# lswzjuer/pytorch-quantity

Measured on NVIDIA B200. Metric: calib images/sec (hist+KL), higher is better.
Workload: dtype f32

## Files before the change

include/pq_sm100.h:

```cpp
#ifndef PQ_SM100_H
#define PQ_SM100_H

#include <stddef.h>
#include <stdint.h>

#ifdef __cplusplus
extern "C" {
#endif

typedef void *pq_stream_t;

#define PQ_VERSION 201

#define PQ_OK 0
#define PQ_EINVAL (-1)
#define PQ_EUNSUPPORTED (-2)
#define PQ_EALIGN (-3)
#define PQ_ETOOMANY (-4)

#define PQ_HIST_BINS 2048
#define PQ_HIST_BINS_MAX 8192
#define PQ_KL_TARGET_BIN 128
#define PQ_KL_CANDIDATES (PQ_HIST_BINS - PQ_KL_TARGET_BIN)
#define PQ_MAX_SEGMENTS 256

int pq_version(void);
const char *pq_error_string(int code);

int pq_absmax_multi_f32(const float *const *xs_host, const uint64_t *ns_host, int k,
                        uint32_t *max_bits, pq_stream_t stream);

int pq_absmax_per_channel_f32(const float *x, uint64_t outer, int channels, uint64_t inner,
                              uint32_t *max_bits, pq_stream_t stream);

int pq_conv_epilogue_f32(float *y, const float *bias, int N, int C, uint64_t hw, float *relu_out,
                         uint32_t *max_slot, pq_stream_t stream);
int pq_eltwise_add_f32(const float *a, const float *b, float *z, size_t n, float *relu_out, uint32_t *max_slot,
                       pq_stream_t stream);

int pq_hist2048_multi_f32(const float *const *xs_host, const uint64_t *ns_host,
                          const float *intervals_host, int k, long long *hist,
                          pq_stream_t stream);

size_t pq_kl_workspace_doubles(void);
int pq_kl_search_f64(const double *counts, int k, double *workspace, double *kl,
                     int *threshold, pq_stream_t stream);

int pq_hist_multi_f32(const float *const *xs_host, const uint64_t *ns_host, const float *intervals_host,
                      int k, int nbins, long long *hist, pq_stream_t stream);
size_t pq_kl_workspace_doubles_n(int nbins);
int pq_kl_search_n_f64(const double *counts, int k, int nbins, double *workspace, double *kl,
                       int *threshold, pq_stream_t stream);

int pq_fakequant_f32(const float *x, float *y, size_t n, int bit, float lo, float hi,
                     int dequant, pq_stream_t stream);

int pq_add_clamp_f32(const float *a, const float *b, float *y, size_t n, float lo, float hi,
                     pq_stream_t stream);

int pq_rshift_f32(const float *x, float *y, size_t n, int rs, float lo, float hi, pq_stream_t stream);

int pq_clamp_scale_f32(const float *x, float *y, size_t n, float lo, float hi, float scale,
                       pq_stream_t stream);

int pq_quantize_nchw_to_nhwc_s8(const float *x, int8_t *q, int N, int C, int H, int W, int c_pad,
                                int ib, pq_stream_t stream);

int pq_quantize_im2col_s8(const float *x, int8_t *a, int N, int C, int H, int W, int R, int S,
                          int stride_h, int stride_w, int pad_h, int pad_w, int kp, int ib,
                          pq_stream_t stream);

int pq_quantize_nchw_to_padded_nhwc8_s8(const float *x, int8_t *q, int N, int C, int H, int W, int pad_h,
                                        int pad_w, int Hp, int Wp, int ib, pq_stream_t stream);

typedef struct pq_conv_desc {
    int N, H, W, C;
    int K;
    int R, S;
    int stride_h, stride_w, pad_h, pad_w;
    int P, Q;
    int rs;
    int ob;
    int dil_h, dil_w;
} pq_conv_desc;

#define PQ_FLAG_RELU 1
#define PQ_FLAG_BIAS_FOLDED 2
#define PQ_FLAG_NO_WINDOWS 4

int pq_gemm_s8(const int8_t *a, const int8_t *w, const int32_t *bias_q, int M, int N, int K, int rs, int ob, int hw,
               int flags, float *out_f32, int8_t *out_s8, pq_stream_t stream);
int pq_conv2d_s8(const int8_t *x_nhwc, const int8_t *w_krsc, const int32_t *bias_q, const pq_conv_desc *desc_host,
                 int flags, float *out_f32_nchw, int8_t *out_s8_nhwc, pq_stream_t stream);

int pq_bias_fold_s32(const int32_t *bias_q, int n, int rs, int32_t *out, pq_stream_t stream);

int pq_quantize_nchw_to_s2d16_s8(const float *x, int8_t *q, int N, int C, int H, int W, int pad_t, int pad_l,
                                 int Hp2, int Wp2, int ib, pq_stream_t stream);

int pq_conv2d_smallc_s8(const int8_t *xp, const int8_t *w_krs8, const int32_t *bias_q,
                        const pq_conv_desc *desc_host, int Hp, int Wp, int flags, float *out_f32_nchw,
                        int8_t *out_s8_nhwc, pq_stream_t stream);

int pq_avgpool_global_nhwc_f32(const void *x, int is16, int bit, int relu, int N, int HW, int C, float *out,
                               pq_stream_t stream);

int pq_relu_s8(const int8_t *x, int8_t *y, size_t n, pq_stream_t stream);

int pq_maxpool_nhwc_s8(const int8_t *x, int8_t *y, int N, int H, int W, int C, int k, int stride, int pad,
                       int relu, pq_stream_t stream);

int pq_add_requant(const void *a, int a_is16, int a_bit, int a_relu, const void *b, int b_is16, int b_bit,
                   int b_relu, size_t n, int flags, int16_t *out16, int8_t *out8, int q_bit, pq_stream_t stream);

#define PQ_CONCAT_MAX_SOURCES 8
typedef struct pq_concat_src {
    const void *ptr;
    int is16;
    int channels;
    int bit;
    int relu;
} pq_concat_src;
int pq_concat_requant_s8(const pq_concat_src *srcs_host, int k, size_t pixels, int q_bit, int c_out_pad,
                         int8_t *out, pq_stream_t stream);

typedef struct pq_add_desc {
    const void *shortcut;
    int shortcut_is16, shortcut_bit, shortcut_relu;
    int out_relu;
    int q_bit;
    int16_t *out16;
    int8_t *out8;
} pq_add_desc;
int pq_conv2d_s8_add(const int8_t *x_nhwc, const int8_t *w_krsc, const int32_t *bias_q, const pq_conv_desc *desc_host,
                     const pq_add_desc *add_host, int flags, pq_stream_t stream);

#ifdef __cplusplus
}
#endif
#endif
```

pytorch-quantity_b200/common/quantity/_native.py:

```python
import ctypes
import os

import numpy as np
import torch

_PKG_ROOT = os.path.dirname(os.path.dirname(os.path.dirname(os.path.abspath(__file__))))
LIB_PATH = os.path.join(_PKG_ROOT, "lib", "libpq_sm100.so")

HIST_BINS = 2048
HIST_BINS_MAX = 8192
KL_TARGET_BIN = 128
KL_CANDIDATES = HIST_BINS - KL_TARGET_BIN
MAX_SEGMENTS = 256
PQ_VERSION = 201

_vp, _i, _sz, _f = ctypes.c_void_p, ctypes.c_int, ctypes.c_size_t, ctypes.c_float
SYMBOLS = {
    "pq_version": (_i, []),
    "pq_error_string": (ctypes.c_char_p, [_i]),
    "pq_absmax_multi_f32": (_i, [_vp, _vp, _i, _vp, _vp]),
    "pq_absmax_per_channel_f32": (_i, [_vp, ctypes.c_uint64, _i, ctypes.c_uint64, _vp, _vp]),
    "pq_conv_epilogue_f32": (_i, [_vp, _vp, _i, _i, ctypes.c_uint64, _vp, _vp, _vp]),
    "pq_eltwise_add_f32": (_i, [_vp, _vp, _vp, _sz, _vp, _vp, _vp]),
    "pq_hist2048_multi_f32": (_i, [_vp, _vp, _vp, _i, _vp, _vp]),
    "pq_kl_workspace_doubles": (_sz, []),
    "pq_kl_search_f64": (_i, [_vp, _i, _vp, _vp, _vp, _vp]),
    "pq_hist_multi_f32": (_i, [_vp, _vp, _vp, _i, _i, _vp, _vp]),
    "pq_kl_workspace_doubles_n": (_sz, [_i]),
    "pq_kl_search_n_f64": (_i, [_vp, _i, _i, _vp, _vp, _vp, _vp]),
    "pq_fakequant_f32": (_i, [_vp, _vp, _sz, _i, _f, _f, _i, _vp]),
    "pq_add_clamp_f32": (_i, [_vp, _vp, _vp, _sz, _f, _f, _vp]),
    "pq_rshift_f32": (_i, [_vp, _vp, _sz, _i, _f, _f, _vp]),
    "pq_clamp_scale_f32": (_i, [_vp, _vp, _sz, _f, _f, _f, _vp]),
    "pq_quantize_nchw_to_nhwc_s8": (_i, [_vp, _vp, _i, _i, _i, _i, _i, _i, _vp]),
    "pq_quantize_im2col_s8": (_i, [_vp, _vp] + [_i] * 12 + [_vp]),
    "pq_quantize_nchw_to_padded_nhwc8_s8": (_i, [_vp, _vp] + [_i] * 9 + [_vp]),
    "pq_conv2d_smallc_s8": (_i, [_vp, _vp, _vp, _vp, _i, _i, _i, _vp, _vp, _vp]),
    "pq_quantize_nchw_to_s2d16_s8": (_i, [_vp, _vp] + [_i] * 9 + [_vp]),
    "pq_gemm_s8": (_i, [_vp, _vp, _vp, _i, _i, _i, _i, _i, _i, _i, _vp, _vp, _vp]),
    "pq_conv2d_s8": (_i, [_vp, _vp, _vp, _vp, _i, _vp, _vp, _vp]),
    "pq_conv2d_s8_add": (_i, [_vp, _vp, _vp, _vp, _vp, _i, _vp]),
    "pq_relu_s8": (_i, [_vp, _vp, _sz, _vp]),
    "pq_maxpool_nhwc_s8": (_i, [_vp, _vp, _i, _i, _i, _i, _i, _i, _i, _i, _vp]),
    "pq_avgpool_global_nhwc_f32": (_i, [_vp, _i, _i, _i, _i, _i, _i, _vp, _vp]),
    "pq_add_requant": (_i, [_vp, _i, _i, _i, _vp, _i, _i, _i, _sz, _i, _vp, _vp, _i, _vp]),
    "pq_concat_requant_s8": (_i, [_vp, _i, _sz, _i, _i, _vp, _vp]),
    "pq_bias_fold_s32": (_i, [_vp, _i, _i, _vp, _vp]),
}
FLAG_RELU = 1
FLAG_BIAS_FOLDED = 2
FLAG_NO_WINDOWS = 4


class ConvDesc(ctypes.Structure):
    _fields_ = [(n, ctypes.c_int) for n in
                ("N", "H", "W", "C", "K", "R", "S", "stride_h", "stride_w", "pad_h", "pad_w",
                 "P", "Q", "rs", "ob", "dil_h", "dil_w")]


class AddDesc(ctypes.Structure):
    _fields_ = [("shortcut", ctypes.c_void_p), ("shortcut_is16", ctypes.c_int), ("shortcut_bit", ctypes.c_int),
                ("shortcut_relu", ctypes.c_int), ("out_relu", ctypes.c_int), ("q_bit", ctypes.c_int),
                ("out16", ctypes.c_void_p), ("out8", ctypes.c_void_p)]


class ConcatSrc(ctypes.Structure):
    _fields_ = [("ptr", ctypes.c_void_p), ("is16", ctypes.c_int), ("channels", ctypes.c_int),
                ("bit", ctypes.c_int), ("relu", ctypes.c_int)]


CONCAT_MAX_SOURCES = 8

_lib = None

LAUNCHES = {"total": 0}
_profile = None


def set_profile(store):
    global _profile
    _profile = store


class _Timed:
    def __init__(self, name, kernels, alg_bytes, device):
        self.name, self.kernels, self.alg_bytes, self.device = name, kernels, alg_bytes, device

    def __enter__(self):
        LAUNCHES["total"] += self.kernels
        LAUNCHES[self.name] = LAUNCHES.get(self.name, 0) + self.kernels
        if _profile is not None:
            self.start = torch.cuda.Event(enable_timing=True)
            self.start.record(torch.cuda.current_stream(self.device))
        return self

    def __exit__(self, *exc):
        if _profile is not None:
            end = torch.cuda.Event(enable_timing=True)
            end.record(torch.cuda.current_stream(self.device))
            _profile.setdefault(self.name, []).append((self.start, end, self.alg_bytes))
        return False


def lib():
    global _lib
    if _lib is None:
        if not os.path.exists(LIB_PATH):
            raise ImportError(
                "libpq_sm100.so not found at %s -- build it with `python __graft_entry__.py` "
                "(or `make -C pytorch-quantity_b200/csrc`).  This package has no CPU fallback." % LIB_PATH)
        handle = ctypes.CDLL(LIB_PATH)
        handle.pq_version.restype, handle.pq_version.argtypes = SYMBOLS["pq_version"]
        if handle.pq_version() != PQ_VERSION:
            raise ImportError(
                "%s is version %d, this package needs %d -- rebuild with `python __graft_entry__.py`"
                % (LIB_PATH, handle.pq_version(), PQ_VERSION))
        for name, (res, args) in SYMBOLS.items():
            fn = getattr(handle, name)
            fn.restype, fn.argtypes = res, args
        _lib = handle
    return _lib


def check(rc, what):
    if rc != 0:
        raise RuntimeError("%s failed: %s (code %d)" % (what, lib().pq_error_string(rc).decode(), rc))


def _stream(t):
    return torch.cuda.current_stream(t.device).cuda_stream


def require_cuda(t, what):
    if not isinstance(t, torch.Tensor) or not t.is_cuda:
        raise RuntimeError("%s needs a CUDA tensor: the B200 path has no CPU fallback" % what)


def to_device_f32(x, device=None):
    if isinstance(x, torch.Tensor):
        t = x.detach()
    else:
        t = torch.from_numpy(np.ascontiguousarray(np.asarray(x)))
    if not t.is_cuda:
        if not torch.cuda.is_available():
            raise RuntimeError("no CUDA device: pytorch-quantity_b200 has no CPU fallback")
        t = t.to(device or "cuda", non_blocking=True)
    if t.dtype != torch.float32:
        t = t.float()
    return t.contiguous().view(-1)


def _seg_arrays(tensors):
    k = len(tensors)
    ptrs = (ctypes.c_void_p * k)(*[t.data_ptr() if t.numel() else 0 for t in tensors])
    ns = (ctypes.c_uint64 * k)(*[t.numel() for t in tensors])
    return ptrs, ns


def absmax_multi(tensors, max_bits):
    for lo in range(0, len(tensors), MAX_SEGMENTS):
        part = tensors[lo:lo + MAX_SEGMENTS]
        ptrs, ns = _seg_arrays(part)
        out = max_bits[lo:lo + len(part)]
        with _Timed("absmax", 1, 4 * sum(t.numel() for t in part), max_bits.device):
            check(lib().pq_absmax_multi_f32(ptrs, ns, len(part), out.data_ptr(), _stream(max_bits)),
                  "pq_absmax_multi_f32")


def absmax_per_channel(x, max_bits, channel_dim=1):
    require_cuda(x, "absmax_per_channel")
    if x.dtype != torch.float32:
        raise RuntimeError("fp32 expected, got %s" % x.dtype)
    xc = x.detach().contiguous()
    shape = tuple(xc.shape)
    channel_dim %= len(shape)
    outer = int(np.prod(shape[:channel_dim], dtype=np.int64))
    inner = int(np.prod(shape[channel_dim + 1:], dtype=np.int64))
    C = shape[channel_dim]
    assert max_bits.dtype == torch.int32 and max_bits.numel() >= C and max_bits.is_contiguous()
    with _Timed("absmax_channel", 1, 4 * xc.numel(), xc.device):
        check(lib().pq_absmax_per_channel_f32(xc.data_ptr() if xc.numel() else None, outer, C, inner,
                                              max_bits.data_ptr(), _stream(xc)), "pq_absmax_per_channel_f32")


def _require_f32_contiguous(tensors, what):
    dev = tensors[0].device
    for t in tensors:
        require_cuda(t, what)
        if t.dtype != torch.float32 or not t.is_contiguous() or t.device != dev:
            raise RuntimeError("%s needs contiguous fp32 tensors on %s, got %s %s on %s"
                               % (what, dev, t.dtype, "contiguous" if t.is_contiguous() else "strided", t.device))


def conv_epilogue(y, bias, relu=False, max_slot=None):
    _require_f32_contiguous((y, bias), "conv_epilogue")
    N, C, H, W = y.shape
    if bias.numel() != C:
        raise RuntimeError("conv_epilogue: %d bias values for %d channels" % (bias.numel(), C))
    r = torch.empty_like(y) if relu else None
    with _Timed("conv_epilogue", 1, y.numel() * (12 if relu else 8), y.device):
        check(lib().pq_conv_epilogue_f32(y.data_ptr(), bias.data_ptr(), N, C, H * W, r.data_ptr() if relu else None,
                                         max_slot, _stream(y)), "pq_conv_epilogue_f32")
    return r


def eltwise_add(a, b, relu=False, max_slot=None):
    _require_f32_contiguous((a, b), "eltwise_add")
    if a.shape != b.shape:
        raise RuntimeError("eltwise_add: shapes %s and %s differ" % (tuple(a.shape), tuple(b.shape)))
    z = torch.empty_like(a)
    r = torch.empty_like(a) if relu else None
    with _Timed("eltwise", 1, a.numel() * (16 if relu else 12), a.device):
        check(lib().pq_eltwise_add_f32(a.data_ptr(), b.data_ptr(), z.data_ptr(), a.numel(),
                                       r.data_ptr() if relu else None, max_slot, _stream(a)),
              "pq_eltwise_add_f32")
    return z, r


def hist_multi(tensors, intervals, hist):
    nbins = int(hist.shape[1])
    for lo in range(0, len(tensors), MAX_SEGMENTS):
        part = tensors[lo:lo + MAX_SEGMENTS]
        ptrs, ns = _seg_arrays(part)
        iv = (ctypes.c_float * len(part))(*[float(v) for v in intervals[lo:lo + len(part)]])
        out = hist[lo:lo + len(part)]
        with _Timed("hist", 1, 4 * sum(t.numel() for t in part), hist.device):
            if nbins == HIST_BINS:
                check(lib().pq_hist2048_multi_f32(ptrs, ns, iv, len(part), out.data_ptr(), _stream(hist)),
                      "pq_hist2048_multi_f32")
            else:
                check(lib().pq_hist_multi_f32(ptrs, ns, iv, len(part), nbins, out.data_ptr(), _stream(hist)),
                      "pq_hist_multi_f32 (INTERVAL_NUM=%d)" % nbins)


def kl_search(counts_f64, want_curves=False):
    require_cuda(counts_f64, "kl_search")
    assert counts_f64.dtype == torch.float64 and counts_f64.dim() == 2
    nbins = int(counts_f64.shape[1])
    counts_f64 = counts_f64.contiguous()
    k = counts_f64.shape[0]
    dev = counts_f64.device
    ws = torch.empty(k * lib().pq_kl_workspace_doubles_n(nbins), dtype=torch.float64, device=dev)
    thr = torch.empty(k, dtype=torch.int32, device=dev)
    kl = torch.empty((k, max(nbins - KL_TARGET_BIN, 0)), dtype=torch.float64, device=dev) if want_curves else None
    with _Timed("kl", 3, 8 * counts_f64.numel(), dev):
        check(lib().pq_kl_search_n_f64(counts_f64.data_ptr(), k, nbins, ws.data_ptr(),
                                       kl.data_ptr() if want_curves else None, thr.data_ptr(),
                                       _stream(counts_f64)), "pq_kl_search_n_f64 (INTERVAL_NUM=%d)" % nbins)
    return thr, kl


def bias_fold(bias_i32, rs):
    require_cuda(bias_i32, "bias_fold")
    n = bias_i32.numel()
    if n % 16 or bias_i32.dtype != torch.int32 or not 1 <= int(rs) <= 20:
        return bias_i32
    out = torch.empty(3 * n, dtype=torch.int32, device=bias_i32.device)
    check(lib().pq_bias_fold_s32(bias_i32.contiguous().data_ptr(), n, int(rs), out.data_ptr(), _stream(bias_i32)),
          "pq_bias_fold_s32")
    return out


def conv_out_size(in_hw, kernel, stride, padding, dilation=(1, 1)):
    return ((in_hw[0] + 2 * padding[0] - (kernel[0] - 1) * dilation[0] - 1) // stride[0] + 1,
            (in_hw[1] + 2 * padding[1] - (kernel[1] - 1) * dilation[1] - 1) // stride[1] + 1)


def _conv_desc(N, H, W, C, K, kernel, stride, padding, rs, ob, dilation=(1, 1)):
    P, Q = conv_out_size((H, W), kernel, stride, padding, dilation)
    return ConvDesc(N, H, W, C, K, kernel[0], kernel[1], stride[0], stride[1], padding[0], padding[1], P, Q,
                    int(rs), int(ob), dilation[0], dilation[1])


def _bias_flags(bias_q, n, relu):
    return (FLAG_RELU if relu else 0) | (FLAG_BIAS_FOLDED if bias_q.numel() == 3 * n else 0)


def _flat_out(x):
    require_cuda(x, "elementwise kernel")
    if x.dtype != torch.float32:
        raise RuntimeError("fp32 expected, got %s" % x.dtype)
    xc = x.contiguous()
    return xc, torch.empty_like(xc)


def fakequant(x, bit, lo=-128.0, hi=127.0, dequant=True):
    xc, y = _flat_out(x)
    with _Timed("fakequant", 1, 8 * xc.numel(), xc.device):
        check(lib().pq_fakequant_f32(xc.data_ptr(), y.data_ptr(), xc.numel(), int(bit), lo, hi,
                                     1 if dequant else 0, _stream(xc)), "pq_fakequant_f32")
    return y


def add_clamp(a, b, lo=-128.0, hi=127.0):
    require_cuda(b, "add_clamp")
    if a.shape != b.shape:
        a, b = torch.broadcast_tensors(a, b)
    ac, y = _flat_out(a)
    bc = b.contiguous()
    with _Timed("add_clamp", 1, 12 * ac.numel(), ac.device):
        check(lib().pq_add_clamp_f32(ac.data_ptr(), bc.data_ptr(), y.data_ptr(), ac.numel(), lo, hi,
                                     _stream(ac)), "pq_add_clamp_f32")
    return y


def rshift(x, rs, lo=-128.0, hi=127.0):
    xc, y = _flat_out(x)
    check(lib().pq_rshift_f32(xc.data_ptr(), y.data_ptr(), xc.numel(), int(rs), lo, hi, _stream(xc)),
          "pq_rshift_f32")
    return y


def clamp_scale(x, lo, hi, scale):
    xc, y = _flat_out(x)
    check(lib().pq_clamp_scale_f32(xc.data_ptr(), y.data_ptr(), xc.numel(), lo, hi, scale, _stream(xc)),
          "pq_clamp_scale_f32")
    return y


def quantize_nchw_to_nhwc_s8(x, ib, c_pad):
    require_cuda(x, "quantize_nchw_to_nhwc_s8")
    assert x.dim() == 4 and x.dtype == torch.float32
    xc = x.contiguous()
    N, C, H, W = xc.shape
    q = torch.empty((N, H, W, c_pad), dtype=torch.int8, device=x.device)
    with _Timed("quantize_s8", 1, xc.numel() * 4 + q.numel(), xc.device):
        check(lib().pq_quantize_nchw_to_nhwc_s8(xc.data_ptr(), q.data_ptr(), N, C, H, W, c_pad, int(ib),
                                                _stream(xc)), "pq_quantize_nchw_to_nhwc_s8")
    return q


def quantize_im2col_s8(x, ib, kernel, stride, padding, kp):
    require_cuda(x, "quantize_im2col_s8")
    assert x.dim() == 4 and x.dtype == torch.float32
    xc = x.contiguous()
    N, C, H, W = xc.shape
    R, S = kernel
    P, Q = conv_out_size((H, W), kernel, stride, padding)
    a = torch.empty((N * P * Q, kp), dtype=torch.int8, device=x.device)
    with _Timed("quantize_s8", 1, xc.numel() * 4 + a.numel(), xc.device):
        check(lib().pq_quantize_im2col_s8(xc.data_ptr(), a.data_ptr(), N, C, H, W, R, S, stride[0], stride[1],
                                          padding[0], padding[1], kp, int(ib), _stream(xc)),
              "pq_quantize_im2col_s8")
    return a, (N, P, Q)


def quantize_pad_nhwc8_s8(x, ib, padding, Hp, Wp):
    require_cuda(x, "quantize_pad_nhwc8_s8")
    assert x.dim() == 4 and x.dtype == torch.float32
    xc = x.contiguous()
    N, C, H, W = xc.shape
    q = torch.empty((N, Hp, Wp, 8), dtype=torch.int8, device=x.device)
    with _Timed("quantize_s8", 1, xc.numel() * 4 + q.numel(), xc.device):
        check(lib().pq_quantize_nchw_to_padded_nhwc8_s8(xc.data_ptr(), q.data_ptr(), N, C, H, W, padding[0],
                                                        padding[1], Hp, Wp, int(ib), _stream(xc)),
              "pq_quantize_nchw_to_padded_nhwc8_s8")
    return q


def quantize_s2d16_s8(x, ib, pad_tl, Hp2, Wp2):
    require_cuda(x, "quantize_s2d16_s8")
    assert x.dim() == 4 and x.dtype == torch.float32
    xc = x.contiguous()
    N, C, H, W = xc.shape
    q = torch.empty((N, Hp2, Wp2, 16), dtype=torch.int8, device=x.device)
    with _Timed("quantize_s8", 1, xc.numel() * 4 + q.numel(), xc.device):
        check(lib().pq_quantize_nchw_to_s2d16_s8(xc.data_ptr(), q.data_ptr(), N, C, H, W, pad_tl[0], pad_tl[1], Hp2, Wp2,
                                                 int(ib), _stream(xc)), "pq_quantize_nchw_to_s2d16_s8")
    return q


def conv2d_smallc_s8(xp, w_krs8, bias_q, in_hw, kernel, stride, padding, rs, ob, want_f32=True, want_s8=False,
                     c_real=None, relu=False, ops=None):
    require_cuda(xp, "conv2d_smallc_s8")
    N, Hp, Wp, _ = xp.shape
    K = w_krs8.shape[0]
    R, S = kernel
    d = _conv_desc(N, in_hw[0], in_hw[1], 8, K, kernel, stride, padding, rs, ob)
    P, Q = d.P, d.Q
    out_f32 = torch.empty((N, K, P, Q), dtype=torch.float32, device=xp.device) if want_f32 else None
    out_s8 = torch.empty((N, P, Q, K), dtype=torch.int8, device=xp.device) if want_s8 else None
    with _Timed("conv_s8", 1, ops or 2 * N * P * Q * K * R * S * (c_real or 8), xp.device):
        check(lib().pq_conv2d_smallc_s8(xp.data_ptr(), w_krs8.data_ptr(), bias_q.data_ptr(), ctypes.byref(d), Hp, Wp,
                                        _bias_flags(bias_q, K, relu), out_f32.data_ptr() if want_f32 else None,
                                        out_s8.data_ptr() if want_s8 else None, _stream(xp)), "pq_conv2d_smallc_s8")
    return out_f32, out_s8


def gemm_s8(a, w, bias_q, rs, ob, hw=1, want_f32=True, want_s8=False, k_real=None, relu=False):
    require_cuda(a, "gemm_s8")
    M, K = a.shape
    N = w.shape[0]
    out_f32 = out_s8 = None
    if want_f32:
        out_f32 = torch.empty((M // hw, N, hw) if hw > 1 else (M, N), dtype=torch.float32, device=a.device)
    if want_s8:
        out_s8 = torch.empty((M, N), dtype=torch.int8, device=a.device)
    with _Timed("gemm_s8", 1, 2 * M * N * (k_real or K), a.device):
        check(lib().pq_gemm_s8(a.data_ptr(), w.data_ptr(), bias_q.data_ptr(), M, N, K, int(rs), int(ob), hw,
                               _bias_flags(bias_q, N, relu), out_f32.data_ptr() if want_f32 else None,
                               out_s8.data_ptr() if want_s8 else None, _stream(a)), "pq_gemm_s8")
    return out_f32, out_s8


def conv2d_s8(x_nhwc, w_krsc, bias_q, stride, padding, rs, ob, want_f32=True, want_s8=False, c_real=None,
              relu=False, dilation=(1, 1), windows=True):
    require_cuda(x_nhwc, "conv2d_s8")
    N, H, W, C = x_nhwc.shape
    K, R, S, C2 = w_krsc.shape
    assert C == C2
    dilation = (int(dilation[0]), int(dilation[1])) if (R, S) != (1, 1) else (1, 1)
    d = _conv_desc(N, H, W, C, K, (R, S), stride, padding, rs, ob, dilation)
    P, Q = d.P, d.Q
    out_f32 = torch.empty((N, K, P, Q), dtype=torch.float32, device=x_nhwc.device) if want_f32 else None
    out_s8 = torch.empty((N, P, Q, K), dtype=torch.int8, device=x_nhwc.device) if want_s8 else None
    with _Timed("conv_s8", 1, 2 * N * P * Q * K * R * S * (c_real or C), x_nhwc.device):
        check(lib().pq_conv2d_s8(x_nhwc.data_ptr(), w_krsc.data_ptr(), bias_q.data_ptr(), ctypes.byref(d),
                                 _bias_flags(bias_q, K, relu) | (0 if windows else FLAG_NO_WINDOWS),
                                 out_f32.data_ptr() if want_f32 else None,
                                 out_s8.data_ptr() if want_s8 else None, _stream(x_nhwc)), "pq_conv2d_s8")
    return out_f32, out_s8


def conv2d_s8_add(x_nhwc, w_krsc, bias_q, stride, padding, rs, ob, shortcut, shortcut_bit, shortcut_relu, q_bit,
                  out_relu, want16=True, c_real=None):
    require_cuda(x_nhwc, "conv2d_s8_add")
    N, H, W, C = x_nhwc.shape
    K, R, S, C2 = w_krsc.shape
    assert C == C2
    d = _conv_desc(N, H, W, C, K, (R, S), stride, padding, rs, ob)
    P, Q = d.P, d.Q
    assert tuple(shortcut.shape) == (N, P, Q, K) and shortcut.is_contiguous()
    out16 = torch.empty((N, P, Q, K), dtype=torch.int16, device=x_nhwc.device) if want16 else None
    out8 = torch.empty((N, P, Q, K), dtype=torch.int8, device=x_nhwc.device)
    add = AddDesc(shortcut.data_ptr(), 1 if shortcut.dtype == torch.int16 else 0, int(shortcut_bit),
                  1 if shortcut_relu else 0, 1 if out_relu else 0, int(q_bit),
                  out16.data_ptr() if want16 else None, out8.data_ptr())
    with _Timed("conv_add_s8", 1, 2 * N * P * Q * K * R * S * (c_real or C), x_nhwc.device):
        check(lib().pq_conv2d_s8_add(x_nhwc.data_ptr(), w_krsc.data_ptr(), bias_q.data_ptr(), ctypes.byref(d),
                                     ctypes.byref(add), _bias_flags(bias_q, K, False), _stream(x_nhwc)),
              "pq_conv2d_s8_add")
    return out16, out8


def relu_s8(x):
    require_cuda(x, "relu_s8")
    xc = x.contiguous()
    y = torch.empty_like(xc)
    with _Timed("relu_s8", 1, 2 * xc.numel(), xc.device):
        check(lib().pq_relu_s8(xc.data_ptr(), y.data_ptr(), xc.numel(), _stream(xc)), "pq_relu_s8")
    return y


def maxpool_nhwc_s8(x, k, stride, pad, relu=False):
    require_cuda(x, "maxpool_nhwc_s8")
    N, H, W, C = x.shape
    P, Q = conv_out_size((H, W), (k, k), (stride, stride), (pad, pad))
    y = torch.empty((N, P, Q, C), dtype=torch.int8, device=x.device)
    with _Timed("maxpool_s8", 1, x.numel() + y.numel(), x.device):
        check(lib().pq_maxpool_nhwc_s8(x.data_ptr(), y.data_ptr(), N, H, W, C, k, stride, pad, 1 if relu else 0,
                                       _stream(x)), "pq_maxpool_nhwc_s8")
    return y


def avgpool_global_nhwc(x, bit, relu=False):
    require_cuda(x, "avgpool_global_nhwc")
    N, H, W, C = x.shape
    is16 = x.dtype == torch.int16
    if C % 8 or H * W * (32768 if is16 else 128) >= (1 << 24) or not x.is_contiguous():
        return None
    y = torch.empty((N, C, 1, 1), dtype=torch.float32, device=x.device)
    with _Timed("avgpool_s8", 1, x.numel() * x.element_size() + y.numel() * 4, x.device):
        check(lib().pq_avgpool_global_nhwc_f32(x.data_ptr(), 1 if is16 else 0, int(bit), 1 if relu else 0, N, H * W, C,
                                               y.data_ptr(), _stream(x)), "pq_avgpool_global_nhwc_f32")
    return y


def add_requant(a, a_bit, a_relu, b, b_bit, b_relu, q_bit, want16=True, want8=True, out_relu=False):
    require_cuda(a, "add_requant")
    assert a.shape == b.shape and a.is_contiguous() and b.is_contiguous()
    out16 = torch.empty(a.shape, dtype=torch.int16, device=a.device) if want16 else None
    out8 = torch.empty(a.shape, dtype=torch.int8, device=a.device) if want8 else None
    nbytes = a.numel() * (a.element_size() + b.element_size() + (2 if want16 else 0) + (1 if want8 else 0))
    with _Timed("add_requant", 1, nbytes, a.device):
        check(lib().pq_add_requant(a.data_ptr(), 1 if a.dtype == torch.int16 else 0, int(a_bit),
                                   1 if a_relu else 0, b.data_ptr(), 1 if b.dtype == torch.int16 else 0,
                                   int(b_bit), 1 if b_relu else 0, a.numel(), FLAG_RELU if out_relu else 0,
                                   out16.data_ptr() if want16 else None, out8.data_ptr() if want8 else None,
                                   int(q_bit), _stream(a)), "pq_add_requant")
    return out16, out8


def concat_requant_s8(sources, q_bit, c_out_pad=None):
    first = sources[0][0]
    require_cuda(first, "concat_requant_s8")
    N, H, W = first.shape[:3]
    k = len(sources)
    if k > CONCAT_MAX_SOURCES:
        raise RuntimeError("concat_requant_s8: at most %d sources" % CONCAT_MAX_SOURCES)
    arr = (ConcatSrc * k)()
    c_sum = nbytes = 0
    for i, (t, bit, relu) in enumerate(sources):
        assert t.is_contiguous() and tuple(t.shape[:3]) == (N, H, W) and t.dtype in (torch.int8, torch.int16)
        arr[i] = ConcatSrc(t.data_ptr(), 1 if t.dtype == torch.int16 else 0, t.shape[3], int(bit), 1 if relu else 0)
        c_sum += t.shape[3]
        nbytes += t.numel() * t.element_size()
    c_out_pad = c_sum if c_out_pad is None else c_out_pad
    out = torch.empty((N, H, W, c_out_pad), dtype=torch.int8, device=first.device)
    with _Timed("concat_requant", 1, nbytes + out.numel(), first.device):
        check(lib().pq_concat_requant_s8(arr, k, N * H * W, int(q_bit), c_out_pad, out.data_ptr(), _stream(first)),
              "pq_concat_requant_s8")
    return out
```

pytorch-quantity_b200/common/quantity/distribution_collector.py:

```python
import numpy as np
import torch

from . import _native


class DistributionCollector:

    def __init__(self, tensor_list, interval_num=2048, statistic=1, worker_num=1, debug=False,
                 device=None):
        if int(interval_num) != interval_num or not (1 <= interval_num <= _native.HIST_BINS_MAX):
            raise ValueError("INTERVAL_NUM must be an integer in [1, %d] (PQ_EUNSUPPORTED beyond: shared-memory "
                             "histogram), got %r" % (_native.HIST_BINS_MAX, interval_num))
        interval_num = int(interval_num)
        self._tensor_list = tensor_list
        self._interval_num = interval_num
        self._statistic = statistic
        self._worker_num = worker_num
        self._debug = debug
        self._device = torch.device(device) if device is not None else None
        self._max_bits = None
        self._hist = None
        self._max_vals = {name: 0 for name in tensor_list}
        self._distributions = {}
        self._max_dirty = False
        self._hist_dirty = False
        self._max_vals_refreshed_flag = False
        self._added_to_distributions_flag = False

    def _ensure_state(self, sample):
        if self._max_bits is not None:
            return
        if self._device is None:
            if isinstance(sample, torch.Tensor) and sample.is_cuda:
                self._device = sample.device
            else:
                if not torch.cuda.is_available():
                    raise RuntimeError("no CUDA device: DistributionCollector has no CPU fallback")
                self._device = torch.device("cuda", torch.cuda.current_device())
        n = len(self._tensor_list)
        self._max_bits = torch.zeros(n, dtype=torch.int32, device=self._device)
        self._hist = torch.zeros((n, self._interval_num), dtype=torch.int64, device=self._device)

    def _gather(self, tensors, skip=()):
        first = next(iter(tensors.values())) if len(tensors) else None
        self._ensure_state(first)
        empty = torch.empty(0, device=self._device) if skip else None
        return [empty if name in skip else _native.to_device_f32(tensors[name], self._device)
                for name in self._tensor_list]

    @property
    def max_vals(self):
        assert self._max_vals_refreshed_flag, "Please use refresh_max_val() first."
        if self._max_dirty:
            vals = self._max_bits.view(torch.float32).cpu().numpy()
            for name, v in zip(self._tensor_list, vals):
                self._max_vals[name] = np.float32(v) if v > 0 else 0
            self._max_dirty = False
        return self._max_vals

    @property
    def distribution_intervals(self):
        assert self._max_vals_refreshed_flag, "Please use refresh_max_val() first."
        max_vals = self.max_vals
        intervals = {}
        for name in self._tensor_list:
            intervals[name] = self._statistic * max_vals[name] / self._interval_num + 1e-12
        self._distribution_intervals = intervals
        return intervals

    @property
    def distributions(self):
        assert self._added_to_distributions_flag, "Please use add_to_distributions() first."
        if self._hist_dirty:
            h = self._hist.cpu().numpy()
            fits = int(h.max(initial=0)) < 2 ** 31
            for i, name in enumerate(self._tensor_list):
                self._distributions[name] = h[i].astype(np.int32) if fits else h[i].copy()
            self._hist_dirty = False
        return self._distributions

    def refresh_max_val(self, tensors):
        self._refresh_max_val_except(tensors, ())

    def _refresh_max_val_except(self, tensors, reduced):
        self._max_vals_refreshed_flag = True
        _native.absmax_multi(self._gather(tensors, reduced), self._max_bits)
        self._max_dirty = True

    def _max_slot(self, name):
        self._ensure_state(None)
        return self._max_bits.data_ptr() + 4 * self._tensor_list.index(name)

    def add_to_distributions(self, tensors):
        if self._debug and self._added_to_distributions_flag:
            return
        self._added_to_distributions_flag = True
        if not hasattr(self, "_distribution_intervals"):
            print("interval:", self.distribution_intervals)
        flat = self._gather(tensors)
        intervals = [np.float32(self._distribution_intervals[name]) for name in self._tensor_list]
        _native.hist_multi(flat, intervals, self._hist)
        self._hist_dirty = True

    def refresh_channel_max_val(self, tensors, channel_dim=1):
        if not hasattr(self, "_chan_bits"):
            self._chan_bits = {}
        for name in self._tensor_list:
            x = tensors[name]
            if not (isinstance(x, torch.Tensor) and x.is_cuda):
                x = _native.to_device_f32(x, self._device).view(np.shape(tensors[name]))
            if x.dim() <= channel_dim:
                continue
            if name not in self._chan_bits:
                self._chan_bits[name] = torch.zeros(x.shape[channel_dim], dtype=torch.int32, device=x.device)
            _native.absmax_per_channel(x.float(), self._chan_bits[name], channel_dim)

    @property
    def channel_max_vals(self):
        assert hasattr(self, "_chan_bits"), "Please use refresh_channel_max_val() first."
        return {name: b.view(torch.float32).cpu().numpy() for name, b in self._chan_bits.items()}

    def all_reduce_channel_max(self, group=None):
        import torch.distributed as dist
        if dist.is_available() and dist.is_initialized() and dist.get_world_size(group) > 1:
            for name in self._tensor_list:
                if name in getattr(self, "_chan_bits", {}):
                    dist.all_reduce(self._chan_bits[name], op=dist.ReduceOp.MAX, group=group)

    def device_state(self):
        return self._max_bits, self._hist

    def all_reduce_max(self, group=None):
        import torch.distributed as dist
        if dist.is_available() and dist.is_initialized() and dist.get_world_size(group) > 1:
            self._ensure_state(None)
            dist.all_reduce(self._max_bits, op=dist.ReduceOp.MAX, group=group)
            self._max_dirty = True
            self._max_vals_refreshed_flag = True

    def all_reduce_hist(self, group=None):
        import torch.distributed as dist
        if dist.is_available() and dist.is_initialized() and dist.get_world_size(group) > 1:
            self._ensure_state(None)
            dist.all_reduce(self._hist, op=dist.ReduceOp.SUM, group=group)
            self._hist_dirty = True
            self._added_to_distributions_flag = True
```

pytorch-quantity_b200/csrc/pq_stats.cu:

```cuda
#include "pq_stats_kernels.cuh"

namespace {

constexpr int kHistCopies = 1;

int build_table(pq::SegTable &t, const float *const *xs, const uint64_t *ns, const float *params, int k)
{
    if (k < 0 || (k > 0 && (!xs || !ns))) return PQ_EINVAL;
    if (k > PQ_MAX_SEGMENTS) return PQ_ETOOMANY;
    unsigned long long total = 0;
    for (int i = 0; i < k; ++i) {
        if (ns[i] && !xs[i]) return PQ_EINVAL;
        if (((unsigned long long)xs[i] & 3ull) != 0) return PQ_EALIGN;
        t.ptr[i] = xs[i];
        t.n[i] = ns[i];
        t.param[i] = params ? params[i] : 0.0f;
        total += pq::seg_num_chunks(xs[i], ns[i]);
        if (total > 0xffffffffull) return PQ_EUNSUPPORTED;
        t.chunk_end[i] = (unsigned int)total;
    }
    t.k = k;
    t.total_chunks = (unsigned int)total;
    return PQ_OK;
}

unsigned int grid_for(unsigned int total_chunks, int ctas_per_sm)
{
    unsigned int g = (unsigned int)(pq::kNumSMs * ctas_per_sm);
    return total_chunks < g ? total_chunks : g;
}

}

extern "C" int pq_absmax_multi_f32(const float *const *xs_host, const uint64_t *ns_host, int k,
                                   uint32_t *max_bits, pq_stream_t stream)
{
    if (k == 0) return PQ_OK;
    if (!max_bits) return PQ_EINVAL;
    pq::SegTable t;
    int rc = build_table(t, xs_host, ns_host, nullptr, k);
    if (rc != PQ_OK) return rc;
    pq::absmax_multi_kernel<<<grid_for(t.total_chunks, 8), pq::kStatThreads, 0, (cudaStream_t)stream>>>(
        t, max_bits);
    return (int)cudaGetLastError();
}

namespace {
void magic31(unsigned int d, unsigned int *m, int *s)
{
    int l = 0;
    while ((1ull << l) < d) ++l;
    *s = 31 + l;
    *m = (unsigned int)(((1ull << *s) + d - 1) / d);
}
}

extern "C" int pq_absmax_per_channel_f32(const float *x, uint64_t outer, int channels, uint64_t inner,
                                         uint32_t *max_bits, pq_stream_t stream)
{
    if (channels < 0) return PQ_EINVAL;
    if (outer == 0 || channels == 0 || inner == 0) return PQ_OK;
    if (!x || !max_bits) return PQ_EINVAL;
    if (((unsigned long long)x & 3ull) != 0) return PQ_EALIGN;
    if (channels > 8192 || inner >= (1ull << 31) - (1ull << 14) || outer * (uint64_t)channels >= (1ull << 31))
        return PQ_EUNSUPPORTED;
    const uint64_t per_img = (uint64_t)channels * inner;
    if (inner < 784 && outer >= 16 && (per_img & 3) == 0 && per_img / 4 < (1ull << 31) && outer < (1ull << 31) &&
        ((unsigned long long)x & 15ull) == 0) {
        const unsigned int vec_per_img = (unsigned int)(per_img / 4);
        const unsigned int gx = (vec_per_img + pq::kStatThreads - 1) / pq::kStatThreads;
        unsigned long long gy = ((unsigned long long)pq::kNumSMs * 8 + gx - 1) / gx;
        if (gy > outer / 2) gy = outer / 2;
        if (gy > 65535) gy = 65535;
        if (gy < 1) gy = 1;
        pq::absmax_periodic_kernel<<<dim3(gx, (unsigned int)gy), pq::kStatThreads, 0, (cudaStream_t)stream>>>(
            reinterpret_cast<const float4 *>(x), vec_per_img, (unsigned int)outer, (unsigned int)inner, max_bits);
        return (int)cudaGetLastError();
    }
    pq::ChannelGeom g;
    g.total = outer * (uint64_t)channels * inner;
    g.inner = (unsigned int)inner;
    g.channels = (unsigned int)channels;
    magic31(g.inner, &g.m_inner, &g.s_inner);
    magic31(g.channels, &g.m_chan, &g.s_chan);
    unsigned long long head = ((16ull - ((unsigned long long)x & 15ull)) & 15ull) >> 2;
    if (head > g.total) head = g.total;
    const unsigned long long nvec = (g.total - head) >> 2;
    const unsigned int tail = (unsigned int)(g.total - head - (nvec << 2));
    unsigned long long chunks = (nvec + pq::kChunkVecs - 1) / pq::kChunkVecs;
    if (chunks == 0) chunks = 1;
    if (chunks > 0xffffffffull) return PQ_EUNSUPPORTED;
    pq::absmax_per_channel_kernel<<<grid_for((unsigned int)chunks, 8), pq::kStatThreads, (size_t)channels * 4,
                                    (cudaStream_t)stream>>>(x, g, (unsigned int)head, nvec, tail,
                                                            (unsigned int)chunks, max_bits);
    return (int)cudaGetLastError();
}

namespace {
bool aligned16(const void *p) { return (((unsigned long long)p) & 15ull) == 0; }

int launch_epilogue(pq::EpiArgs &p, int mode, cudaStream_t stream)
{
    const unsigned long long nvec = p.n >> 2;
    if (nvec >= (1ull << 31) || (mode == pq::EPI_BIAS1 && p.n >= (1ull << 31))) return PQ_EUNSUPPORTED;
    magic31(p.hw, &p.m_hw, &p.s_hw);
    magic31(p.channels, &p.m_chan, &p.s_chan);
    unsigned long long blocks = (nvec / pq::kEpiUnroll + pq::kStatThreads - 1) / pq::kStatThreads;
    if (blocks > (unsigned long long)pq::kNumSMs * 8) blocks = (unsigned long long)pq::kNumSMs * 8;
    if (blocks == 0) blocks = 1;
    const unsigned int g = (unsigned int)blocks;
    if (mode == pq::EPI_BIAS4) pq::epilogue_kernel<pq::EPI_BIAS4><<<g, pq::kStatThreads, 0, stream>>>(p);
    else if (mode == pq::EPI_BIAS1) pq::epilogue_kernel<pq::EPI_BIAS1><<<g, pq::kStatThreads, 0, stream>>>(p);
    else pq::epilogue_kernel<pq::EPI_ADD><<<g, pq::kStatThreads, 0, stream>>>(p);
    return (int)cudaGetLastError();
}
}

extern "C" int pq_conv_epilogue_f32(float *y, const float *bias, int N, int C, uint64_t hw, float *relu_out,
                                    uint32_t *max_slot, pq_stream_t stream)
{
    if (N < 0 || C <= 0) return PQ_EINVAL;
    if (N == 0 || hw == 0) return PQ_OK;
    if (!y || !bias || relu_out == y) return PQ_EINVAL;
    if (!aligned16(y) || !aligned16(relu_out) || (((unsigned long long)bias) & 3ull)) return PQ_EALIGN;
    if (hw >= (1ull << 31) || (uint64_t)N * (uint64_t)C >= (1ull << 31)) return PQ_EUNSUPPORTED;
    pq::EpiArgs p = {};
    p.a = y;
    p.b = bias;
    p.out = y;
    p.relu_out = relu_out;
    p.max_slot = max_slot;
    p.n = (uint64_t)N * (uint64_t)C * hw;
    p.channels = (unsigned int)C;
    const int mode = (hw & 3) == 0 ? pq::EPI_BIAS4 : pq::EPI_BIAS1;
    p.hw = (unsigned int)(mode == pq::EPI_BIAS4 ? hw / 4 : hw);
    return launch_epilogue(p, mode, (cudaStream_t)stream);
}

extern "C" int pq_eltwise_add_f32(const float *a, const float *b, float *z, size_t n, float *relu_out,
                                  uint32_t *max_slot, pq_stream_t stream)
{
    if (n == 0) return PQ_OK;
    if (!a || !b || !z || z == a || z == b || relu_out == a || relu_out == b || relu_out == z) return PQ_EINVAL;
    if (!aligned16(a) || !aligned16(b) || !aligned16(z) || !aligned16(relu_out)) return PQ_EALIGN;
    pq::EpiArgs p = {};
    p.a = a;
    p.b = b;
    p.out = z;
    p.relu_out = relu_out;
    p.max_slot = max_slot;
    p.n = n;
    p.hw = 1;
    p.channels = 1;
    return launch_epilogue(p, pq::EPI_ADD, (cudaStream_t)stream);
}

extern "C" int pq_hist2048_multi_f32(const float *const *xs_host, const uint64_t *ns_host,
                                     const float *intervals_host, int k, long long *hist,
                                     pq_stream_t stream)
{
    if (k == 0) return PQ_OK;
    if (!hist || !intervals_host) return PQ_EINVAL;
    for (int i = 0; i < k; ++i)
        if (!(intervals_host[i] > 0.0f)) return PQ_EINVAL;
    pq::SegTable t;
    int rc = build_table(t, xs_host, ns_host, intervals_host, k);
    if (rc != PQ_OK) return rc;
    constexpr size_t smem = pq::hist_smem_bytes(kHistCopies);
    auto kern = pq::hist_multi_kernel<kHistCopies>;
    static bool attr_set = false;
    if (!attr_set) {
        PQ_CUDA_TRY(cudaFuncSetAttribute(kern, cudaFuncAttributeMaxDynamicSharedMemorySize, (int)smem));
        attr_set = true;
    }
    const int ctas_per_sm = (int)((200 * 1024) / smem) < 8 ? (int)((200 * 1024) / smem) : 8;
    kern<<<grid_for(t.total_chunks, ctas_per_sm), pq::kStatThreads, smem, (cudaStream_t)stream>>>(
        t, reinterpret_cast<unsigned long long *>(hist));
    return (int)cudaGetLastError();
}

extern "C" int pq_hist_multi_f32(const float *const *xs_host, const uint64_t *ns_host, const float *intervals_host,
                                 int k, int nbins, long long *hist, pq_stream_t stream)
{
    if (nbins == PQ_HIST_BINS) return pq_hist2048_multi_f32(xs_host, ns_host, intervals_host, k, hist, stream);
    if (nbins < 1) return PQ_EINVAL;
    if (nbins > PQ_HIST_BINS_MAX) return PQ_EUNSUPPORTED;
    if (k == 0) return PQ_OK;
    if (!hist || !intervals_host) return PQ_EINVAL;
    for (int i = 0; i < k; ++i)
        if (!(intervals_host[i] > 0.0f)) return PQ_EINVAL;
    pq::SegTable t;
    int rc = build_table(t, xs_host, ns_host, intervals_host, k);
    if (rc != PQ_OK) return rc;
    const size_t smem = (size_t)nbins * 4;
    static bool attr_set = false;
    if (!attr_set) {
        PQ_CUDA_TRY(cudaFuncSetAttribute(pq::hist_generic_kernel, cudaFuncAttributeMaxDynamicSharedMemorySize,
                                         PQ_HIST_BINS_MAX * 4));
        attr_set = true;
    }
    int ctas_per_sm = (int)((200 * 1024) / (smem + 1024));
    ctas_per_sm = ctas_per_sm < 1 ? 1 : (ctas_per_sm > 8 ? 8 : ctas_per_sm);
    pq::hist_generic_kernel<<<grid_for(t.total_chunks, ctas_per_sm), pq::kStatThreads, smem, (cudaStream_t)stream>>>(
        t, nbins, reinterpret_cast<unsigned long long *>(hist));
    return (int)cudaGetLastError();
}
```

pytorch-quantity_b200/csrc/pq_stats_kernels.cuh:

```cuda
#pragma once
#include "pq_common.cuh"

namespace pq {

constexpr int kStatThreads = 256;
constexpr int kVecPerThread = 8;
constexpr int kChunkVecs = kStatThreads * kVecPerThread;
constexpr int kChunkElems = kChunkVecs * 4;

struct SegGeom {
    const float *p;
    unsigned long long n;
    unsigned int head;
    unsigned long long nvec;
    const float4 *body;
    unsigned int tail;
};

__device__ __forceinline__ SegGeom seg_geom(const SegTable &t, int s)
{
    SegGeom g;
    g.p = t.ptr[s];
    g.n = t.n[s];
    unsigned long long addr = (unsigned long long)g.p;
    unsigned long long head = ((16ull - (addr & 15ull)) & 15ull) >> 2;
    g.head = (unsigned int)(head < g.n ? head : g.n);
    g.nvec = (g.n - g.head) >> 2;
    g.body = reinterpret_cast<const float4 *>(g.p + g.head);
    g.tail = (unsigned int)(g.n - g.head - (g.nvec << 2));
    return g;
}

__host__ __device__ inline unsigned int seg_num_chunks(const float *p, unsigned long long n)
{
    unsigned long long addr = (unsigned long long)p;
    unsigned long long head = ((16ull - (addr & 15ull)) & 15ull) >> 2;
    if (head > n) head = n;
    unsigned long long nvec = (n - head) >> 2;
    unsigned long long c = (nvec + kChunkVecs - 1) / kChunkVecs;
    return (unsigned int)(c ? c : 1);
}

__device__ __forceinline__ unsigned int absbits(float v) { return __float_as_uint(v) & 0x7fffffffu; }

__device__ __forceinline__ void block_max_publish(unsigned int m, unsigned int *s_warp, unsigned int *dst)
{
    m = __reduce_max_sync(0xffffffffu, m);
    if ((threadIdx.x & 31) == 0) s_warp[threadIdx.x >> 5] = m;
    __syncthreads();
    if (threadIdx.x < 32) {
        unsigned int w = threadIdx.x < kStatThreads / 32 ? s_warp[threadIdx.x] : 0u;
        w = __reduce_max_sync(0xffffffffu, w);
        if (threadIdx.x == 0 && w != 0) atomicMax(dst, w);
    }
    __syncthreads();
}

__global__ void __launch_bounds__(kStatThreads)
absmax_multi_kernel(const __grid_constant__ SegTable tab, unsigned int *__restrict__ max_bits)
{
    __shared__ unsigned int s_warp[kStatThreads / 32];
    const unsigned int per = (tab.total_chunks + gridDim.x - 1) / gridDim.x;
    unsigned int c = blockIdx.x * per;
    const unsigned int c_end = min(c + per, tab.total_chunks);
    if (c >= c_end) return;

    int seg = seg_of_chunk(tab, c);
    unsigned int m = 0;
    while (c < c_end) {
        const SegGeom g = seg_geom(tab, seg);
        const unsigned int seg_first = seg ? tab.chunk_end[seg - 1] : 0;
        const unsigned int seg_last = min(tab.chunk_end[seg], c_end);
        for (; c < seg_last; ++c) {
            const unsigned long long v0 = (unsigned long long)(c - seg_first) * kChunkVecs;
            const float4 *src = g.body + v0;
            const unsigned long long left = g.nvec > v0 ? g.nvec - v0 : 0;
            if (left >= (unsigned long long)kChunkVecs) {
                float4 v[kVecPerThread];
#pragma unroll
                for (int i = 0; i < kVecPerThread; ++i) v[i] = ld_stream_f4(src + threadIdx.x + i * kStatThreads);
#pragma unroll
                for (int i = 0; i < kVecPerThread; ++i)
                    m = max(max(m, max(absbits(v[i].x), absbits(v[i].y))), max(absbits(v[i].z), absbits(v[i].w)));
            } else {
                for (unsigned int i = threadIdx.x; i < (unsigned int)left; i += kStatThreads) {
                    float4 v = ld_stream_f4(src + i);
                    m = max(max(m, max(absbits(v.x), absbits(v.y))), max(absbits(v.z), absbits(v.w)));
                }
            }
            if (c == seg_first) {
                if (threadIdx.x < g.head) m = max(m, absbits(g.p[threadIdx.x]));
                if (threadIdx.x < g.tail) m = max(m, absbits(g.p[g.n - g.tail + threadIdx.x]));
            }
        }
        block_max_publish(m, s_warp, max_bits + seg);
        m = 0;
        ++seg;
    }
}

struct ChannelGeom {
    unsigned long long total;
    unsigned int inner, channels;
    unsigned int m_inner, m_chan;
    int s_inner, s_chan;
};

__device__ __forceinline__ unsigned int magic_div(unsigned int n, unsigned int m, int s)
{
    return (unsigned int)(((unsigned long long)n * m) >> s);
}

__device__ __forceinline__ void chan_add_straddle(unsigned int *smax, const float4 &v, unsigned int rem, unsigned int ch,
                                                  const ChannelGeom &g)
{
    const float e[4] = {v.x, v.y, v.z, v.w};
#pragma unroll
    for (int j = 0; j < 4; ++j) {
        while (rem >= g.inner) {
            rem -= g.inner;
            if (++ch == g.channels) ch = 0;
        }
        atomicMax(smax + ch, absbits(e[j]));
        ++rem;
    }
}

__global__ void __launch_bounds__(kStatThreads)
absmax_per_channel_kernel(const float *__restrict__ x, const ChannelGeom g, unsigned int head,
                          unsigned long long nvec, unsigned int tail, unsigned int total_chunks,
                          unsigned int *__restrict__ max_bits)
{
    extern __shared__ unsigned int s_cmax[];
    const unsigned int per = (total_chunks + gridDim.x - 1) / gridDim.x;
    unsigned int c = blockIdx.x * per;
    const unsigned int c_end = min(c + per, total_chunks);
    if (c >= c_end) return;
    for (unsigned int i = threadIdx.x; i < g.channels; i += kStatThreads) s_cmax[i] = 0;
    __syncthreads();

    const float4 *body = reinterpret_cast<const float4 *>(x + head);
    const unsigned long long e0 = (unsigned long long)head + (unsigned long long)c * kChunkElems;
    const unsigned long long p0 = e0 / g.inner;
    unsigned int r0 = (unsigned int)(e0 - p0 * g.inner);
    unsigned int ch0 = (unsigned int)(p0 % g.channels);

    for (; c < c_end; ++c) {
        const unsigned long long v0 = (unsigned long long)c * kChunkVecs;
        const float4 *src = body + v0;
        const unsigned long long left = nvec > v0 ? nvec - v0 : 0;
        if (left >= (unsigned long long)kChunkVecs) {
            float4 v[kVecPerThread];
#pragma unroll
            for (int i = 0; i < kVecPerThread; ++i) v[i] = ld_stream_f4(src + threadIdx.x + i * kStatThreads);
#pragma unroll
            for (int i = 0; i < kVecPerThread; ++i) {
                const unsigned int r = r0 + 4u * (threadIdx.x + i * kStatThreads);
                const unsigned int q = magic_div(r, g.m_inner, g.s_inner);
                const unsigned int rem = r - q * g.inner;
                unsigned int ch = ch0 + q;
                ch -= magic_div(ch, g.m_chan, g.s_chan) * g.channels;
                const unsigned int m4 = max(max(absbits(v[i].x), absbits(v[i].y)), max(absbits(v[i].z), absbits(v[i].w)));
                const bool whole = rem + 3u < g.inner;
                int same;
                __match_all_sync(0xffffffffu, ch, &same);
                if (same && __all_sync(0xffffffffu, whole)) {
                    const unsigned int m = __reduce_max_sync(0xffffffffu, m4);
                    if ((threadIdx.x & 31) == 0) atomicMax(s_cmax + ch, m);
                } else if (whole) {
                    atomicMax(s_cmax + ch, m4);
                } else {
                    chan_add_straddle(s_cmax, v[i], rem, ch, g);
                }
            }
        } else {
            for (unsigned int i = threadIdx.x; i < (unsigned int)left; i += kStatThreads) {
                const float4 w = ld_stream_f4(src + i);
                const unsigned int r = r0 + 4u * i;
                const unsigned int q = magic_div(r, g.m_inner, g.s_inner);
                unsigned int ch = ch0 + q;
                ch -= magic_div(ch, g.m_chan, g.s_chan) * g.channels;
                chan_add_straddle(s_cmax, w, r - q * g.inner, ch, g);
            }
        }
        r0 += kChunkElems;
        const unsigned int q = magic_div(r0, g.m_inner, g.s_inner);
        r0 -= q * g.inner;
        ch0 += q;
        ch0 -= magic_div(ch0, g.m_chan, g.s_chan) * g.channels;
    }
    if (blockIdx.x == 0 && threadIdx.x == 0) {
        for (unsigned int j = 0; j < head + tail; ++j) {
            const unsigned long long e = j < head ? j : g.total - tail + (j - head);
            atomicMax(s_cmax + (unsigned int)((e / g.inner) % g.channels), absbits(x[e]));
        }
    }
    __syncthreads();
    for (unsigned int i = threadIdx.x; i < g.channels; i += kStatThreads) {
        const unsigned int m = s_cmax[i];
        if (m) atomicMax(max_bits + i, m);
    }
}

constexpr int kPerRows = 8;

__global__ void __launch_bounds__(kStatThreads)
absmax_periodic_kernel(const float4 *__restrict__ x, unsigned int vec_per_img, unsigned int images, unsigned int inner,
                       unsigned int *__restrict__ max_bits)
{
    __shared__ unsigned int s_cmax[kStatThreads * 4 + 2];
    for (unsigned int i = threadIdx.x; i < kStatThreads * 4 + 2; i += kStatThreads) s_cmax[i] = 0;
    __syncthreads();
    const unsigned int j = blockIdx.x * kStatThreads + threadIdx.x;
    const unsigned int ch_base = (blockIdx.x * kStatThreads * 4u) / inner;
    if (j < vec_per_img) {
        unsigned int m0 = 0, m1 = 0, m2 = 0, m3 = 0;
        const unsigned int step = gridDim.y;
        unsigned int r = blockIdx.y;
        for (; r + (kPerRows - 1) * step < images; r += kPerRows * step) {
            float4 v[kPerRows];
#pragma unroll
            for (int i = 0; i < kPerRows; ++i) v[i] = ld_stream_f4(x + (size_t)(r + i * step) * vec_per_img + j);
#pragma unroll
            for (int i = 0; i < kPerRows; ++i) {
                m0 = max(m0, absbits(v[i].x)); m1 = max(m1, absbits(v[i].y));
                m2 = max(m2, absbits(v[i].z)); m3 = max(m3, absbits(v[i].w));
            }
        }
        for (; r < images; r += step) {
            const float4 w = ld_stream_f4(x + (size_t)r * vec_per_img + j);
            m0 = max(m0, absbits(w.x)); m1 = max(m1, absbits(w.y)); m2 = max(m2, absbits(w.z)); m3 = max(m3, absbits(w.w));
        }
        const unsigned int e = 4u * j;
        atomicMax(s_cmax + (e / inner - ch_base), m0);
        atomicMax(s_cmax + ((e + 1u) / inner - ch_base), m1);
        atomicMax(s_cmax + ((e + 2u) / inner - ch_base), m2);
        atomicMax(s_cmax + ((e + 3u) / inner - ch_base), m3);
    }
    __syncthreads();
    for (unsigned int i = threadIdx.x; i < kStatThreads * 4 + 2; i += kStatThreads) {
        const unsigned int m = s_cmax[i];
        if (m) atomicMax(max_bits + ch_base + i, m);
    }
}

enum EpiMode { EPI_BIAS4 = 0, EPI_BIAS1 = 1, EPI_ADD = 2 };
constexpr int kEpiUnroll = 4;

struct EpiArgs {
    const float *a;
    const float *b;
    float *out;
    float *relu_out;
    unsigned int *max_slot;
    unsigned long long n;
    unsigned int hw, channels;
    unsigned int m_hw, m_chan;
    int s_hw, s_chan;
};

__device__ __forceinline__ float relu_aten(float v) { return isnan(v) ? v : fmaxf(v, 0.0f); }

template <int MODE>
__device__ __forceinline__ float4 epi_load_a(const EpiArgs &p, unsigned int i)
{
    return MODE == EPI_ADD ? ld_stream_f4(reinterpret_cast<const float4 *>(p.a) + i)
                           : __ldcs(reinterpret_cast<const float4 *>(p.a) + i);
}

template <int MODE>
__device__ __forceinline__ float4 epi_load_b(const EpiArgs &p, unsigned int i)
{
    if (MODE == EPI_ADD) return ld_stream_f4(reinterpret_cast<const float4 *>(p.b) + i);
    if (MODE == EPI_BIAS4) {
        const unsigned int plane = magic_div(i, p.m_hw, p.s_hw);
        const unsigned int c = plane - magic_div(plane, p.m_chan, p.s_chan) * p.channels;
        const float v = __ldg(p.b + c);
        return make_float4(v, v, v, v);
    }
    const unsigned int e = 4u * i;
    const unsigned int plane = magic_div(e, p.m_hw, p.s_hw);
    unsigned int rem = e - plane * p.hw;
    unsigned int c = plane - magic_div(plane, p.m_chan, p.s_chan) * p.channels;
    float v[4];
#pragma unroll
    for (int j = 0; j < 4; ++j) {
        v[j] = __ldg(p.b + c);
        if (++rem == p.hw) {
            rem = 0;
            if (++c == p.channels) c = 0;
        }
    }
    return make_float4(v[0], v[1], v[2], v[3]);
}

__device__ __forceinline__ void epi_store(const EpiArgs &p, unsigned int i, const float4 &a, const float4 &b,
                                          unsigned int &m)
{
    const float4 o = make_float4(__fadd_rn(a.x, b.x), __fadd_rn(a.y, b.y), __fadd_rn(a.z, b.z), __fadd_rn(a.w, b.w));
    __stcs(reinterpret_cast<float4 *>(p.out) + i, o);
    if (p.relu_out)
        reinterpret_cast<float4 *>(p.relu_out)[i] = make_float4(relu_aten(o.x), relu_aten(o.y), relu_aten(o.z),
                                                                relu_aten(o.w));
    m = max(max(m, max(absbits(o.x), absbits(o.y))), max(absbits(o.z), absbits(o.w)));
}

template <int MODE>
__global__ void __launch_bounds__(kStatThreads)
epilogue_kernel(const EpiArgs p)
{
    __shared__ unsigned int s_warp[kStatThreads / 32];
    const unsigned int nvec = (unsigned int)(p.n >> 2);
    const unsigned int stride = gridDim.x * kStatThreads;
    unsigned int i = blockIdx.x * kStatThreads + threadIdx.x;
    unsigned int m = 0;
    for (; i + (kEpiUnroll - 1) * stride < nvec; i += kEpiUnroll * stride) {
        float4 a[kEpiUnroll], b[kEpiUnroll];
#pragma unroll
        for (int u = 0; u < kEpiUnroll; ++u) a[u] = epi_load_a<MODE>(p, i + u * stride);
#pragma unroll
        for (int u = 0; u < kEpiUnroll; ++u) b[u] = epi_load_b<MODE>(p, i + u * stride);
#pragma unroll
        for (int u = 0; u < kEpiUnroll; ++u) epi_store(p, i + u * stride, a[u], b[u], m);
    }
    for (; i < nvec; i += stride) epi_store(p, i, epi_load_a<MODE>(p, i), epi_load_b<MODE>(p, i), m);
    const unsigned long long t = ((unsigned long long)nvec << 2) + blockIdx.x * kStatThreads + threadIdx.x;
    if (t < p.n) {
        float b;
        if (MODE == EPI_ADD) b = p.b[t];
        else b = __ldg(p.b + (unsigned int)((t / (MODE == EPI_BIAS4 ? 4ull * p.hw : p.hw)) % p.channels));
        const float o = __fadd_rn(p.a[t], b);
        p.out[t] = o;
        if (p.relu_out) p.relu_out[t] = relu_aten(o);
        m = max(m, absbits(o));
    }
    if (p.max_slot) block_max_publish(m, s_warp, p.max_slot);
}

struct HistDiv {
    float d;
    float r;
};

__device__ __forceinline__ HistDiv make_hist_div(float interval)
{
    HistDiv h;
    h.d = interval;
    h.r = __frcp_rn(interval);
    return h;
}

__device__ __forceinline__ void hist_add_exact(unsigned int *sh, float v, float interval)
{
    if (v != 0.0f) {
        const float q = __fdiv_rn(fabsf(v), interval);
        const int idx = q >= 2047.0f ? 2047 : (int)q;
        atomicAdd(sh + idx, 1u);
    }
}

constexpr unsigned int kSlowThreshold = 0xff800000u;

__device__ __forceinline__ unsigned int hist_fast_bits(float v, const HistDiv &h)
{
    const float q0 = fminf(__fmul_rn(fabsf(v), h.r), 2047.5f);
    return __float_as_uint(__fadd_rz(q0, 2048.0f));
}

__device__ __forceinline__ bool hist_is_slow(unsigned int bits)
{
    return (bits * 0x100000u - 0x400000u) >= kSlowThreshold;
}

__device__ __forceinline__ unsigned int hist_fast_addr(unsigned int bits, unsigned int base_addr)
{
    return ((bits >> 10) & 0x1ffcu) | base_addr;
}

template <bool ZERO_AWARE>
__device__ __forceinline__ bool hist_add_fast(unsigned int base_addr, unsigned int trash_addr, float v,
                                              const HistDiv &h)
{
    const unsigned int bits = hist_fast_bits(v, h);
    const bool slow = hist_is_slow(bits);
    unsigned int addr = hist_fast_addr(bits, base_addr);
    if (ZERO_AWARE) addr = slow ? trash_addr : addr;
    asm volatile("red.shared.add.u32 [%0], 1;" ::"r"(addr) : "memory");
    return ZERO_AWARE ? (slow && v != 0.0f) : slow;
}

template <bool ZERO_AWARE>
__device__ __forceinline__ void hist_redo(unsigned int *sh, unsigned int base_addr, float v, const HistDiv &h)
{
    const unsigned int bits = hist_fast_bits(v, h);
    if (!hist_is_slow(bits)) return;
    if ((bits & 0x7ffffcu) == 0u) {
        if (v == 0.0f) {
            if (!ZERO_AWARE)
                asm volatile("red.shared.add.u32 [%0], -1;" ::"r"(hist_fast_addr(bits, base_addr)) : "memory");
        } else if (ZERO_AWARE) {
            asm volatile("red.shared.add.u32 [%0], 1;" ::"r"(hist_fast_addr(bits, base_addr)) : "memory");
        }
        return;
    }
    if (!ZERO_AWARE)
        asm volatile("red.shared.add.u32 [%0], -1;" ::"r"(hist_fast_addr(bits, base_addr)) : "memory");
    hist_add_exact(sh, v, h.d);
}

template <bool ZERO_AWARE, int VPT>
__device__ __forceinline__ unsigned int hist_add_vecs(unsigned int base_addr, unsigned int trash_addr,
                                                      const float4 (&v)[VPT], const HistDiv &h)
{
    unsigned int redo = 0;
#pragma unroll
    for (int i = 0; i < VPT; ++i) {
        const bool s0 = hist_add_fast<ZERO_AWARE>(base_addr, trash_addr, v[i].x, h);
        const bool s1 = hist_add_fast<ZERO_AWARE>(base_addr, trash_addr, v[i].y, h);
        const bool s2 = hist_add_fast<ZERO_AWARE>(base_addr, trash_addr, v[i].z, h);
        const bool s3 = hist_add_fast<ZERO_AWARE>(base_addr, trash_addr, v[i].w, h);
        if (s0 | s1 | s2 | s3) redo |= 1u << i;
    }
    return redo;
}

template <bool ZERO_AWARE>
__device__ __forceinline__ void hist_redo_vecs(unsigned int redo, unsigned int *mine, unsigned int mine_addr,
                                               const float4 *psrc, const HistDiv &h)
{
    while (redo) {
        const int slot = __ffs(redo) - 1;
        redo &= redo - 1;
        const float4 w = psrc[threadIdx.x + slot * kStatThreads];
        hist_redo<ZERO_AWARE>(mine, mine_addr, w.x, h);
        hist_redo<ZERO_AWARE>(mine, mine_addr, w.y, h);
        hist_redo<ZERO_AWARE>(mine, mine_addr, w.z, h);
        hist_redo<ZERO_AWARE>(mine, mine_addr, w.w, h);
    }
}

__device__ __forceinline__ bool hist_flagged_has_zero(unsigned int redo, const float4 *psrc)
{
    bool z = false;
    while (redo) {
        const int slot = __ffs(redo) - 1;
        redo &= redo - 1;
        const float4 w = psrc[threadIdx.x + slot * kStatThreads];
        z = z || w.x == 0.0f || w.y == 0.0f || w.z == 0.0f || w.w == 0.0f;
    }
    return z;
}

constexpr size_t hist_smem_bytes(int copies) { return 8192 + (size_t)copies * PQ_HIST_BINS * 4 + 128; }

template <int COPIES, int VPT = kVecPerThread>
__global__ void __launch_bounds__(kStatThreads, VPT <= 4 ? 6 : 4)
hist_multi_kernel(const __grid_constant__ SegTable tab, unsigned long long *__restrict__ hist)
{
    extern __shared__ unsigned int s_raw[];
    const unsigned int raw_addr = (unsigned int)__cvta_generic_to_shared(s_raw);
    const unsigned int pad = ((8192u - (raw_addr & 8191u)) & 8191u) >> 2;
    unsigned int *s_hist = s_raw + pad;
    const unsigned int per = (tab.total_chunks + gridDim.x - 1) / gridDim.x;
    unsigned int c = blockIdx.x * per;
    const unsigned int c_end = min(c + per, tab.total_chunks);
    if (c >= c_end) return;

    for (int i = threadIdx.x; i < COPIES * PQ_HIST_BINS; i += kStatThreads) s_hist[i] = 0;
    __syncthreads();
    unsigned int *mine = s_hist + ((threadIdx.x >> 5) % COPIES) * PQ_HIST_BINS;
    const unsigned int mine_addr = (unsigned int)__cvta_generic_to_shared(mine);
    const unsigned int trash_addr = (unsigned int)__cvta_generic_to_shared(s_hist + COPIES * PQ_HIST_BINS);

    int seg = seg_of_chunk(tab, c);
    bool zero_aware = false;
    while (c < c_end) {
        const SegGeom g = seg_geom(tab, seg);
        const float interval = tab.param[seg];
        const HistDiv hd = make_hist_div(interval);
        const unsigned int seg_first = seg ? tab.chunk_end[seg - 1] : 0;
        const unsigned int seg_last = min(tab.chunk_end[seg], c_end);
        for (; c < seg_last; ++c) {
            const unsigned long long v0 = (unsigned long long)(c - seg_first) * kChunkVecs;
            const float4 *src = g.body + v0;
            const unsigned long long left = g.nvec > v0 ? g.nvec - v0 : 0;
            if (left >= (unsigned long long)kChunkVecs) {
#pragma unroll 1
                for (int part = 0; part < kVecPerThread / VPT; ++part) {
                    const float4 *psrc = src + part * VPT * kStatThreads;
                    float4 v[VPT];
#pragma unroll
                    for (int i = 0; i < VPT; ++i) v[i] = ld_stream_f4(psrc + threadIdx.x + i * kStatThreads);
                    if (zero_aware) {
                        const unsigned int redo = hist_add_vecs<true, VPT>(mine_addr, trash_addr, v, hd);
                        hist_redo_vecs<true>(redo, mine, mine_addr, psrc, hd);
                    } else {
                        const unsigned int redo = hist_add_vecs<false, VPT>(mine_addr, trash_addr, v, hd);
                        bool many_zeros = false;
                        if (__popc(redo) >= 3) many_zeros = hist_flagged_has_zero(redo, psrc);
                        zero_aware = __any_sync(0xffffffffu, many_zeros);
                        hist_redo_vecs<false>(redo, mine, mine_addr, psrc, hd);
                    }
                }
            } else {
                for (unsigned int i = threadIdx.x; i < (unsigned int)left; i += kStatThreads) {
                    const float4 v = ld_stream_f4(src + i);
                    hist_add_exact(mine, v.x, interval);
                    hist_add_exact(mine, v.y, interval);
                    hist_add_exact(mine, v.z, interval);
                    hist_add_exact(mine, v.w, interval);
                }
            }
            if (c == seg_first) {
                if (threadIdx.x < g.head) hist_add_exact(mine, g.p[threadIdx.x], interval);
                if (threadIdx.x < g.tail) hist_add_exact(mine, g.p[g.n - g.tail + threadIdx.x], interval);
            }
        }
        __syncthreads();
        unsigned long long *out = hist + (size_t)seg * PQ_HIST_BINS;
        for (int b = threadIdx.x; b < PQ_HIST_BINS; b += kStatThreads) {
            unsigned int cnt = 0;
#pragma unroll
            for (int k = 0; k < COPIES; ++k) {
                cnt += s_hist[k * PQ_HIST_BINS + b];
                s_hist[k * PQ_HIST_BINS + b] = 0;
            }
            if (cnt) atomicAdd(out + b, (unsigned long long)cnt);
        }
        __syncthreads();
        ++seg;
    }
}

__device__ __forceinline__ void hist_add_exact_n(unsigned int *sh, float v, float interval, int nbins)
{
    if (v != 0.0f) {
        const float q = __fdiv_rn(fabsf(v), interval);
        const int idx = q >= (float)(nbins - 1) ? nbins - 1 : (int)q;
        atomicAdd(sh + idx, 1u);
    }
}

__global__ void __launch_bounds__(kStatThreads)
hist_generic_kernel(const __grid_constant__ SegTable tab, int nbins, unsigned long long *__restrict__ hist)
{
    extern __shared__ unsigned int s_bins[];
    const unsigned int per = (tab.total_chunks + gridDim.x - 1) / gridDim.x;
    unsigned int c = blockIdx.x * per;
    const unsigned int c_end = min(c + per, tab.total_chunks);
    if (c >= c_end) return;
    for (int i = threadIdx.x; i < nbins; i += kStatThreads) s_bins[i] = 0;
    __syncthreads();
    int seg = seg_of_chunk(tab, c);
    while (c < c_end) {
        const SegGeom g = seg_geom(tab, seg);
        const float interval = tab.param[seg];
        const unsigned int seg_first = seg ? tab.chunk_end[seg - 1] : 0;
        const unsigned int seg_last = min(tab.chunk_end[seg], c_end);
        for (; c < seg_last; ++c) {
            const unsigned long long v0 = (unsigned long long)(c - seg_first) * kChunkVecs;
            const float4 *src = g.body + v0;
            const unsigned long long left = g.nvec > v0 ? g.nvec - v0 : 0;
            const unsigned int nv = left >= (unsigned long long)kChunkVecs ? (unsigned int)kChunkVecs : (unsigned int)left;
            for (unsigned int i = threadIdx.x; i < nv; i += 4 * kStatThreads) {
                float4 v[4];
#pragma unroll
                for (int j = 0; j < 4; ++j)
                    if (i + j * kStatThreads < nv) v[j] = ld_stream_f4(src + i + j * kStatThreads);
#pragma unroll
                for (int j = 0; j < 4; ++j)
                    if (i + j * kStatThreads < nv) {
                        hist_add_exact_n(s_bins, v[j].x, interval, nbins);
                        hist_add_exact_n(s_bins, v[j].y, interval, nbins);
                        hist_add_exact_n(s_bins, v[j].z, interval, nbins);
                        hist_add_exact_n(s_bins, v[j].w, interval, nbins);
                    }
            }
            if (c == seg_first) {
                if (threadIdx.x < g.head) hist_add_exact_n(s_bins, g.p[threadIdx.x], interval, nbins);
                if (threadIdx.x < g.tail) hist_add_exact_n(s_bins, g.p[g.n - g.tail + threadIdx.x], interval, nbins);
            }
        }
        __syncthreads();
        unsigned long long *out = hist + (size_t)seg * nbins;
        for (int b = threadIdx.x; b < nbins; b += kStatThreads) {
            const unsigned int cnt = s_bins[b];
            s_bins[b] = 0;
            if (cnt) atomicAdd(out + b, (unsigned long long)cnt);
        }
        __syncthreads();
        ++seg;
    }
}

}
```

Before: 3702.

## Defer conv bias into consumers: fused bias+relu+maxpool, add-with-bias, biased histogram

```diff
diff --git a/include/pq_sm100.h b/include/pq_sm100.h
--- a/include/pq_sm100.h
+++ b/include/pq_sm100.h
@@ -10,7 +10,7 @@
 
 typedef void *pq_stream_t;
 
-#define PQ_VERSION 201
+#define PQ_VERSION 203
 
 #define PQ_OK 0
 #define PQ_EINVAL (-1)
@@ -38,6 +38,14 @@
 int pq_eltwise_add_f32(const float *a, const float *b, float *z, size_t n, float *relu_out, uint32_t *max_slot,
                        pq_stream_t stream);
 
+int pq_conv_bias_relu_f32(const float *y0, const float *bias, int N, int C, uint64_t hw, float *relu_out,
+                          uint32_t *max_slot, pq_stream_t stream);
+int pq_conv_bias_relu_maxpool_f32(const float *y0, const float *bias, int N, int C, int H, int W, float *out,
+                                  uint32_t *max_slot, pq_stream_t stream);
+int pq_eltwise_add_bias_f32(const float *a, const float *bias_a, const float *b, const float *bias_b, int N, int C,
+                            uint64_t hw, float *z, float *relu_out, uint32_t *max_a, uint32_t *max_b,
+                            uint32_t *max_z, pq_stream_t stream);
+
 int pq_hist2048_multi_f32(const float *const *xs_host, const uint64_t *ns_host,
                           const float *intervals_host, int k, long long *hist,
                           pq_stream_t stream);
@@ -48,6 +56,9 @@
 
 int pq_hist_multi_f32(const float *const *xs_host, const uint64_t *ns_host, const float *intervals_host,
                       int k, int nbins, long long *hist, pq_stream_t stream);
+int pq_hist_multi_bias_f32(const float *const *xs_host, const uint64_t *ns_host, const float *intervals_host,
+                           const float *const *biases_host, const int *channels_host, const uint64_t *hw_host,
+                           int k, int nbins, long long *hist, pq_stream_t stream);
 size_t pq_kl_workspace_doubles_n(int nbins);
 int pq_kl_search_n_f64(const double *counts, int k, int nbins, double *workspace, double *kl,
                        int *threshold, pq_stream_t stream);
diff --git a/pytorch-quantity_b200/common/quantity/_native.py b/pytorch-quantity_b200/common/quantity/_native.py
--- a/pytorch-quantity_b200/common/quantity/_native.py
+++ b/pytorch-quantity_b200/common/quantity/_native.py
@@ -12,7 +12,7 @@
 KL_TARGET_BIN = 128
 KL_CANDIDATES = HIST_BINS - KL_TARGET_BIN
 MAX_SEGMENTS = 256
-PQ_VERSION = 201
+PQ_VERSION = 203
 
 _vp, _i, _sz, _f = ctypes.c_void_p, ctypes.c_int, ctypes.c_size_t, ctypes.c_float
 SYMBOLS = {
@@ -22,10 +22,14 @@
     "pq_absmax_per_channel_f32": (_i, [_vp, ctypes.c_uint64, _i, ctypes.c_uint64, _vp, _vp]),
     "pq_conv_epilogue_f32": (_i, [_vp, _vp, _i, _i, ctypes.c_uint64, _vp, _vp, _vp]),
     "pq_eltwise_add_f32": (_i, [_vp, _vp, _vp, _sz, _vp, _vp, _vp]),
+    "pq_conv_bias_relu_f32": (_i, [_vp, _vp, _i, _i, ctypes.c_uint64, _vp, _vp, _vp]),
+    "pq_conv_bias_relu_maxpool_f32": (_i, [_vp, _vp, _i, _i, _i, _i, _vp, _vp, _vp]),
+    "pq_eltwise_add_bias_f32": (_i, [_vp, _vp, _vp, _vp, _i, _i, ctypes.c_uint64, _vp, _vp, _vp, _vp, _vp, _vp]),
     "pq_hist2048_multi_f32": (_i, [_vp, _vp, _vp, _i, _vp, _vp]),
     "pq_kl_workspace_doubles": (_sz, []),
     "pq_kl_search_f64": (_i, [_vp, _i, _vp, _vp, _vp, _vp]),
     "pq_hist_multi_f32": (_i, [_vp, _vp, _vp, _i, _i, _vp, _vp]),
+    "pq_hist_multi_bias_f32": (_i, [_vp, _vp, _vp, _vp, _vp, _vp, _i, _i, _vp, _vp]),
     "pq_kl_workspace_doubles_n": (_sz, [_i]),
     "pq_kl_search_n_f64": (_i, [_vp, _i, _i, _vp, _vp, _vp, _vp]),
     "pq_fakequant_f32": (_i, [_vp, _vp, _sz, _i, _f, _f, _i, _vp]),
@@ -83,12 +87,15 @@
 
 
 class _Timed:
-    def __init__(self, name, kernels, alg_bytes, device):
-        self.name, self.kernels, self.alg_bytes, self.device = name, kernels, alg_bytes, device
+
+    def __init__(self, name, kernels, alg_bytes, device, also=None):
+        self.name, self.kernels, self.alg_bytes, self.device, self.also = name, kernels, alg_bytes, device, also
 
     def __enter__(self):
         LAUNCHES["total"] += self.kernels
         LAUNCHES[self.name] = LAUNCHES.get(self.name, 0) + self.kernels
+        for name, count in (self.also or {}).items():
+            LAUNCHES[name] = LAUNCHES.get(name, 0) + count
         if _profile is not None:
             self.start = torch.cuda.Event(enable_timing=True)
             self.start.record(torch.cuda.current_stream(self.device))
@@ -217,20 +224,71 @@
     return z, r
 
 
-def hist_multi(tensors, intervals, hist):
+def conv_bias_relu(y0, bias, max_slot=None, out=None):
+    _require_f32_contiguous((y0, bias), "conv_bias_relu")
+    N, C, H, W = y0.shape
+    if bias.numel() != C:
+        raise RuntimeError("conv_bias_relu: %d bias values for %d channels" % (bias.numel(), C))
+    if out is not None:
+        _require_f32_contiguous((y0, out), "conv_bias_relu")
+        if out.shape != y0.shape:
+            raise RuntimeError("conv_bias_relu: out is %s, y0 %s" % (tuple(out.shape), tuple(y0.shape)))
+    r = torch.empty_like(y0) if out is None else out
+    with _Timed("conv_epilogue", 1, y0.numel() * 8, y0.device):
+        check(lib().pq_conv_bias_relu_f32(y0.data_ptr(), bias.data_ptr(), N, C, H * W, r.data_ptr(), max_slot,
+                                          _stream(y0)), "pq_conv_bias_relu_f32")
+    return r
+
+
+def conv_bias_relu_maxpool(y0, bias, max_slot=None):
+    _require_f32_contiguous((y0, bias), "conv_bias_relu_maxpool")
+    N, C, H, W = y0.shape
+    if bias.numel() != C:
+        raise RuntimeError("conv_bias_relu_maxpool: %d bias values for %d channels" % (bias.numel(), C))
+    out = torch.empty((N, C, (H - 1) // 2 + 1, (W - 1) // 2 + 1), dtype=torch.float32, device=y0.device)
+    with _Timed("stem_pool", 1, (y0.numel() + out.numel()) * 4, y0.device, also={"conv_epilogue": 1}):
+        check(lib().pq_conv_bias_relu_maxpool_f32(y0.data_ptr(), bias.data_ptr(), N, C, H, W, out.data_ptr(), max_slot,
+                                                  _stream(y0)), "pq_conv_bias_relu_maxpool_f32")
+    return out
+
+
+def eltwise_add_bias(a, bias_a, b, bias_b, relu=False, max_a=None, max_b=None, max_z=None):
+    _require_f32_contiguous([t for t in (a, b, bias_a, bias_b) if t is not None], "eltwise_add_bias")
+    if a.shape != b.shape or a.dim() != 4:
+        raise RuntimeError("eltwise_add_bias: shapes %s and %s differ or are not NCHW" % (tuple(a.shape),
+                                                                                       tuple(b.shape)))
+    N, C, H, W = a.shape
+    for bias in (bias_a, bias_b):
+        if bias is not None and bias.numel() != C:
+            raise RuntimeError("eltwise_add_bias: %d bias values for %d channels" % (bias.numel(), C))
+    z = torch.empty_like(a)
+    r = torch.empty_like(a) if relu else None
+    deferred = (bias_a is not None) + (bias_b is not None)
+    with _Timed("eltwise", 1, a.numel() * (16 if relu else 12), a.device, also={"conv_epilogue": deferred}):
+        check(lib().pq_eltwise_add_bias_f32(a.data_ptr(), None if bias_a is None else bias_a.data_ptr(), b.data_ptr(),
+                                            None if bias_b is None else bias_b.data_ptr(), N, C, H * W, z.data_ptr(),
+                                            r.data_ptr() if relu else None, max_a, max_b, max_z, _stream(a)),
+              "pq_eltwise_add_bias_f32")
+    return z, r
+
+
+def hist_multi(tensors, intervals, hist, biases=None):
     nbins = int(hist.shape[1])
     for lo in range(0, len(tensors), MAX_SEGMENTS):
         part = tensors[lo:lo + MAX_SEGMENTS]
+        k = len(part)
         ptrs, ns = _seg_arrays(part)
-        iv = (ctypes.c_float * len(part))(*[float(v) for v in intervals[lo:lo + len(part)]])
-        out = hist[lo:lo + len(part)]
+        iv = (ctypes.c_float * k)(*[float(v) for v in intervals[lo:lo + k]])
+        out = hist[lo:lo + k]
+        bs = biases[lo:lo + k] if biases is not None else [None] * k
+        bias_ptrs = chans = hws = None
+        if any(b is not None for b in bs):
+            bias_ptrs = (ctypes.c_void_p * k)(*[None if b is None else b[0].data_ptr() for b in bs])
+            chans = (ctypes.c_int * k)(*[0 if b is None else int(b[1]) for b in bs])
+            hws = (ctypes.c_uint64 * k)(*[0 if b is None else int(b[2]) for b in bs])
         with _Timed("hist", 1, 4 * sum(t.numel() for t in part), hist.device):
-            if nbins == HIST_BINS:
-                check(lib().pq_hist2048_multi_f32(ptrs, ns, iv, len(part), out.data_ptr(), _stream(hist)),
-                      "pq_hist2048_multi_f32")
-            else:
-                check(lib().pq_hist_multi_f32(ptrs, ns, iv, len(part), nbins, out.data_ptr(), _stream(hist)),
-                      "pq_hist_multi_f32 (INTERVAL_NUM=%d)" % nbins)
+            check(lib().pq_hist_multi_bias_f32(ptrs, ns, iv, bias_ptrs, chans, hws, k, nbins, out.data_ptr(),
+                                               _stream(hist)), "pq_hist_multi_bias_f32 (INTERVAL_NUM=%d)" % nbins)
 
 
 def kl_search(counts_f64, want_curves=False):
diff --git a/pytorch-quantity_b200/common/quantity/distribution_collector.py b/pytorch-quantity_b200/common/quantity/distribution_collector.py
--- a/pytorch-quantity_b200/common/quantity/distribution_collector.py
+++ b/pytorch-quantity_b200/common/quantity/distribution_collector.py
@@ -91,7 +91,7 @@
         self._ensure_state(None)
         return self._max_bits.data_ptr() + 4 * self._tensor_list.index(name)
 
-    def add_to_distributions(self, tensors):
+    def add_to_distributions(self, tensors, biases=None):
         if self._debug and self._added_to_distributions_flag:
             return
         self._added_to_distributions_flag = True
@@ -99,7 +99,18 @@
             print("interval:", self.distribution_intervals)
         flat = self._gather(tensors)
         intervals = [np.float32(self._distribution_intervals[name]) for name in self._tensor_list]
-        _native.hist_multi(flat, intervals, self._hist)
+        per_tensor = None
+        if biases:
+            per_tensor = [None] * len(self._tensor_list)
+            for i, name in enumerate(self._tensor_list):
+                if name in biases:
+                    t = tensors[name]
+                    if not (isinstance(t, torch.Tensor) and t.is_cuda and t.dim() == 4 and t.is_contiguous()
+                            and t.dtype == torch.float32):
+                        raise RuntimeError("add_to_distributions: biased tensor %r must be a contiguous fp32 CUDA "
+                                           "NCHW tensor" % name)
+                    per_tensor[i] = (biases[name], t.shape[1], t.shape[2] * t.shape[3])
+        _native.hist_multi(flat, intervals, self._hist, per_tensor)
         self._hist_dirty = True
 
     def refresh_channel_max_val(self, tensors, channel_dim=1):
diff --git a/pytorch-quantity_b200/csrc/pq_stats.cu b/pytorch-quantity_b200/csrc/pq_stats.cu
--- a/pytorch-quantity_b200/csrc/pq_stats.cu
+++ b/pytorch-quantity_b200/csrc/pq_stats.cu
@@ -102,7 +102,8 @@
 int launch_epilogue(pq::EpiArgs &p, int mode, cudaStream_t stream)
 {
     const unsigned long long nvec = p.n >> 2;
-    if (nvec >= (1ull << 31) || (mode == pq::EPI_BIAS1 && p.n >= (1ull << 31))) return PQ_EUNSUPPORTED;
+    if (nvec >= (1ull << 31) || ((mode == pq::EPI_BIAS1 || mode == pq::EPI_ADD_BIAS1) && p.n >= (1ull << 31)))
+        return PQ_EUNSUPPORTED;
     magic31(p.hw, &p.m_hw, &p.s_hw);
     magic31(p.channels, &p.m_chan, &p.s_chan);
     unsigned long long blocks = (nvec / pq::kEpiUnroll + pq::kStatThreads - 1) / pq::kStatThreads;
@@ -111,7 +112,9 @@
     const unsigned int g = (unsigned int)blocks;
     if (mode == pq::EPI_BIAS4) pq::epilogue_kernel<pq::EPI_BIAS4><<<g, pq::kStatThreads, 0, stream>>>(p);
     else if (mode == pq::EPI_BIAS1) pq::epilogue_kernel<pq::EPI_BIAS1><<<g, pq::kStatThreads, 0, stream>>>(p);
-    else pq::epilogue_kernel<pq::EPI_ADD><<<g, pq::kStatThreads, 0, stream>>>(p);
+    else if (mode == pq::EPI_ADD) pq::epilogue_kernel<pq::EPI_ADD><<<g, pq::kStatThreads, 0, stream>>>(p);
+    else if (mode == pq::EPI_ADD_BIAS4) pq::epilogue_kernel<pq::EPI_ADD_BIAS4><<<g, pq::kStatThreads, 0, stream>>>(p);
+    else pq::epilogue_kernel<pq::EPI_ADD_BIAS1><<<g, pq::kStatThreads, 0, stream>>>(p);
     return (int)cudaGetLastError();
 }
 }
@@ -137,6 +140,72 @@
     return launch_epilogue(p, mode, (cudaStream_t)stream);
 }
 
+extern "C" int pq_conv_bias_relu_f32(const float *y0, const float *bias, int N, int C, uint64_t hw, float *relu_out,
+                                     uint32_t *max_slot, pq_stream_t stream)
+{
+    if (N < 0 || C <= 0) return PQ_EINVAL;
+    if (N == 0 || hw == 0) return PQ_OK;
+    if (!y0 || !bias || !relu_out || relu_out == y0) return PQ_EINVAL;
+    if (!aligned16(y0) || !aligned16(relu_out) || (((unsigned long long)bias) & 3ull)) return PQ_EALIGN;
+    if (hw >= (1ull << 31) || (uint64_t)N * (uint64_t)C >= (1ull << 31)) return PQ_EUNSUPPORTED;
+    pq::EpiArgs p = {};
+    p.a = y0;
+    p.b = bias;
+    p.out = nullptr;
+    p.relu_out = relu_out;
+    p.max_slot = max_slot;
+    p.n = (uint64_t)N * (uint64_t)C * hw;
+    p.channels = (unsigned int)C;
+    const int mode = (hw & 3) == 0 ? pq::EPI_BIAS4 : pq::EPI_BIAS1;
+    p.hw = (unsigned int)(mode == pq::EPI_BIAS4 ? hw / 4 : hw);
+    return launch_epilogue(p, mode, (cudaStream_t)stream);
+}
+
+extern "C" int pq_eltwise_add_bias_f32(const float *a, const float *bias_a, const float *b, const float *bias_b,
+                                       int N, int C, uint64_t hw, float *z, float *relu_out, uint32_t *max_a,
+                                       uint32_t *max_b, uint32_t *max_z, pq_stream_t stream)
+{
+    if (N < 0 || C <= 0) return PQ_EINVAL;
+    if (N == 0 || hw == 0) return PQ_OK;
+    if (!a || !b || !z || z == a || z == b || relu_out == a || relu_out == b || relu_out == z) return PQ_EINVAL;
+    if (!aligned16(a) || !aligned16(b) || !aligned16(z) || !aligned16(relu_out)) return PQ_EALIGN;
+    if ((((unsigned long long)bias_a) & 3ull) || (((unsigned long long)bias_b) & 3ull)) return PQ_EALIGN;
+    if (hw >= (1ull << 31) || (uint64_t)N * (uint64_t)C >= (1ull << 31)) return PQ_EUNSUPPORTED;
+    pq::EpiArgs p = {};
+    p.a = a;
+    p.b = b;
+    p.out = z;
+    p.relu_out = relu_out;
+    p.max_slot = max_z;
+    p.bias_a = bias_a;
+    p.bias_b = bias_b;
+    p.max_a = max_a;
+    p.max_b = max_b;
+    p.n = (uint64_t)N * (uint64_t)C * hw;
+    p.channels = (unsigned int)C;
+    const int mode = (hw & 3) == 0 ? pq::EPI_ADD_BIAS4 : pq::EPI_ADD_BIAS1;
+    p.hw = (unsigned int)(mode == pq::EPI_ADD_BIAS4 ? hw / 4 : hw);
+    return launch_epilogue(p, mode, (cudaStream_t)stream);
+}
+
+extern "C" int pq_conv_bias_relu_maxpool_f32(const float *y0, const float *bias, int N, int C, int H, int W, float *out,
+                                             uint32_t *max_slot, pq_stream_t stream)
+{
+    if (N < 0 || C <= 0 || H <= 0 || W <= 0) return PQ_EINVAL;
+    if (N == 0) return PQ_OK;
+    if (!y0 || !bias || !out || out == y0) return PQ_EINVAL;
+    if ((((unsigned long long)y0) | ((unsigned long long)out) | ((unsigned long long)bias)) & 3ull) return PQ_EALIGN;
+    if ((uint64_t)N * (uint64_t)C >= (1ull << 31) || (uint64_t)H * (uint64_t)W >= (1ull << 31)) return PQ_EUNSUPPORTED;
+    const int P = (H - 1) / 2 + 1, Q = (W - 1) / 2 + 1;
+    const unsigned long long total = (unsigned long long)N * C * P * Q;
+    if (total >= (1ull << 31)) return PQ_EUNSUPPORTED;
+    unsigned long long blocks = (total + pq::kStatThreads - 1) / pq::kStatThreads;
+    if (blocks > (unsigned long long)pq::kNumSMs * 16) blocks = (unsigned long long)pq::kNumSMs * 16;
+    pq::stem_pool_kernel<<<(unsigned int)blocks, pq::kStatThreads, 0, (cudaStream_t)stream>>>(
+        y0, bias, out, max_slot, (unsigned int)(N * C), (unsigned int)C, H, W, P, Q);
+    return (int)cudaGetLastError();
+}
+
 extern "C" int pq_eltwise_add_f32(const float *a, const float *b, float *z, size_t n, float *relu_out,
                                   uint32_t *max_slot, pq_stream_t stream)
 {
@@ -155,34 +224,11 @@
     return launch_epilogue(p, pq::EPI_ADD, (cudaStream_t)stream);
 }
 
-extern "C" int pq_hist2048_multi_f32(const float *const *xs_host, const uint64_t *ns_host,
-                                     const float *intervals_host, int k, long long *hist,
-                                     pq_stream_t stream)
-{
-    if (k == 0) return PQ_OK;
-    if (!hist || !intervals_host) return PQ_EINVAL;
-    for (int i = 0; i < k; ++i)
-        if (!(intervals_host[i] > 0.0f)) return PQ_EINVAL;
-    pq::SegTable t;
-    int rc = build_table(t, xs_host, ns_host, intervals_host, k);
-    if (rc != PQ_OK) return rc;
-    constexpr size_t smem = pq::hist_smem_bytes(kHistCopies);
-    auto kern = pq::hist_multi_kernel<kHistCopies>;
-    static bool attr_set = false;
-    if (!attr_set) {
-        PQ_CUDA_TRY(cudaFuncSetAttribute(kern, cudaFuncAttributeMaxDynamicSharedMemorySize, (int)smem));
-        attr_set = true;
-    }
-    const int ctas_per_sm = (int)((200 * 1024) / smem) < 8 ? (int)((200 * 1024) / smem) : 8;
-    kern<<<grid_for(t.total_chunks, ctas_per_sm), pq::kStatThreads, smem, (cudaStream_t)stream>>>(
-        t, reinterpret_cast<unsigned long long *>(hist));
-    return (int)cudaGetLastError();
-}
-
-extern "C" int pq_hist_multi_f32(const float *const *xs_host, const uint64_t *ns_host, const float *intervals_host,
-                                 int k, int nbins, long long *hist, pq_stream_t stream)
-{
-    if (nbins == PQ_HIST_BINS) return pq_hist2048_multi_f32(xs_host, ns_host, intervals_host, k, hist, stream);
+namespace {
+int launch_hist(const float *const *xs_host, const uint64_t *ns_host, const float *intervals_host,
+                const float *const *biases_host, const int *channels_host, const uint64_t *hw_host, int k, int nbins,
+                long long *hist, cudaStream_t stream)
+{
     if (nbins < 1) return PQ_EINVAL;
     if (nbins > PQ_HIST_BINS_MAX) return PQ_EUNSUPPORTED;
     if (k == 0) return PQ_OK;
@@ -192,6 +238,39 @@
     pq::SegTable t;
     int rc = build_table(t, xs_host, ns_host, intervals_host, k);
     if (rc != PQ_OK) return rc;
+    pq::SegBias sb;
+    for (int i = 0; i < k; ++i) {
+        const float *bias = biases_host ? biases_host[i] : nullptr;
+        sb.bias[i] = ns_host[i] ? bias : nullptr;
+        if (!sb.bias[i]) continue;
+        if (!channels_host || !hw_host || channels_host[i] <= 0 || hw_host[i] == 0) return PQ_EINVAL;
+        if (((unsigned long long)bias & 3ull) != 0) return PQ_EALIGN;
+        const uint64_t plane = (uint64_t)channels_host[i] * hw_host[i];
+        if (ns_host[i] % plane != 0) return PQ_EINVAL;
+        if (ns_host[i] >= (1ull << 31)) return PQ_EUNSUPPORTED;
+        const bool per4 = (hw_host[i] & 3) == 0 && ((unsigned long long)xs_host[i] & 15ull) == 0;
+        sb.per4[i] = per4 ? 1 : 0;
+        sb.hwq[i] = (unsigned int)(per4 ? hw_host[i] / 4 : hw_host[i]);
+        sb.channels[i] = (unsigned int)channels_host[i];
+        int s_hw, s_chan;
+        magic31(sb.hwq[i], &sb.m_hw[i], &s_hw);
+        magic31(sb.channels[i], &sb.m_chan[i], &s_chan);
+        sb.s_hw[i] = (unsigned char)s_hw;
+        sb.s_chan[i] = (unsigned char)s_chan;
+    }
+    if (nbins == PQ_HIST_BINS) {
+        constexpr size_t smem = pq::hist_smem_bytes(kHistCopies);
+        auto kern = pq::hist_multi_kernel<kHistCopies>;
+        static bool attr_set = false;
+        if (!attr_set) {
+            PQ_CUDA_TRY(cudaFuncSetAttribute(kern, cudaFuncAttributeMaxDynamicSharedMemorySize, (int)smem));
+            attr_set = true;
+        }
+        const int ctas_per_sm = (int)((200 * 1024) / smem) < 8 ? (int)((200 * 1024) / smem) : 8;
+        kern<<<grid_for(t.total_chunks, ctas_per_sm), pq::kStatThreads, smem, stream>>>(
+            t, sb, reinterpret_cast<unsigned long long *>(hist));
+        return (int)cudaGetLastError();
+    }
     const size_t smem = (size_t)nbins * 4;
     static bool attr_set = false;
     if (!attr_set) {
@@ -201,7 +280,32 @@
     }
     int ctas_per_sm = (int)((200 * 1024) / (smem + 1024));
     ctas_per_sm = ctas_per_sm < 1 ? 1 : (ctas_per_sm > 8 ? 8 : ctas_per_sm);
-    pq::hist_generic_kernel<<<grid_for(t.total_chunks, ctas_per_sm), pq::kStatThreads, smem, (cudaStream_t)stream>>>(
-        t, nbins, reinterpret_cast<unsigned long long *>(hist));
-    return (int)cudaGetLastError();
-}
+    pq::hist_generic_kernel<<<grid_for(t.total_chunks, ctas_per_sm), pq::kStatThreads, smem, stream>>>(
+        t, sb, nbins, reinterpret_cast<unsigned long long *>(hist));
+    return (int)cudaGetLastError();
+}
+}
+
+extern "C" int pq_hist2048_multi_f32(const float *const *xs_host, const uint64_t *ns_host,
+                                     const float *intervals_host, int k, long long *hist,
+                                     pq_stream_t stream)
+{
+    return launch_hist(xs_host, ns_host, intervals_host, nullptr, nullptr, nullptr, k, PQ_HIST_BINS, hist,
+                       (cudaStream_t)stream);
+}
+
+extern "C" int pq_hist_multi_f32(const float *const *xs_host, const uint64_t *ns_host, const float *intervals_host,
+                                 int k, int nbins, long long *hist, pq_stream_t stream)
+{
+    return launch_hist(xs_host, ns_host, intervals_host, nullptr, nullptr, nullptr, k, nbins, hist,
+                       (cudaStream_t)stream);
+}
+
+extern "C" int pq_hist_multi_bias_f32(const float *const *xs_host, const uint64_t *ns_host,
+                                      const float *intervals_host, const float *const *biases_host,
+                                      const int *channels_host, const uint64_t *hw_host, int k, int nbins,
+                                      long long *hist, pq_stream_t stream)
+{
+    return launch_hist(xs_host, ns_host, intervals_host, biases_host, channels_host, hw_host, k, nbins, hist,
+                       (cudaStream_t)stream);
+}
diff --git a/pytorch-quantity_b200/csrc/pq_stats_kernels.cuh b/pytorch-quantity_b200/csrc/pq_stats_kernels.cuh
--- a/pytorch-quantity_b200/csrc/pq_stats_kernels.cuh
+++ b/pytorch-quantity_b200/csrc/pq_stats_kernels.cuh
@@ -244,7 +244,7 @@
     }
 }
 
-enum EpiMode { EPI_BIAS4 = 0, EPI_BIAS1 = 1, EPI_ADD = 2 };
+enum EpiMode { EPI_BIAS4 = 0, EPI_BIAS1 = 1, EPI_ADD = 2, EPI_ADD_BIAS4 = 3, EPI_ADD_BIAS1 = 4 };
 constexpr int kEpiUnroll = 4;
 
 struct EpiArgs {
@@ -253,6 +253,8 @@
     float *out;
     float *relu_out;
     unsigned int *max_slot;
+    const float *bias_a, *bias_b;
+    unsigned int *max_a, *max_b;
     unsigned long long n;
     unsigned int hw, channels;
     unsigned int m_hw, m_chan;
@@ -261,48 +263,88 @@
 
 __device__ __forceinline__ float relu_aten(float v) { return isnan(v) ? v : fmaxf(v, 0.0f); }
 
-template <int MODE>
-__device__ __forceinline__ float4 epi_load_a(const EpiArgs &p, unsigned int i)
-{
-    return MODE == EPI_ADD ? ld_stream_f4(reinterpret_cast<const float4 *>(p.a) + i)
-                           : __ldcs(reinterpret_cast<const float4 *>(p.a) + i);
-}
-
-template <int MODE>
-__device__ __forceinline__ float4 epi_load_b(const EpiArgs &p, unsigned int i)
-{
-    if (MODE == EPI_ADD) return ld_stream_f4(reinterpret_cast<const float4 *>(p.b) + i);
-    if (MODE == EPI_BIAS4) {
+__device__ __forceinline__ float4 add4(const float4 &a, const float4 &b)
+{
+    return make_float4(__fadd_rn(a.x, b.x), __fadd_rn(a.y, b.y), __fadd_rn(a.z, b.z), __fadd_rn(a.w, b.w));
+}
+
+__device__ __forceinline__ unsigned int absmax4(unsigned int m, const float4 &o)
+{
+    return max(max(m, max(absbits(o.x), absbits(o.y))), max(absbits(o.z), absbits(o.w)));
+}
+
+template <bool PER4>
+__device__ __forceinline__ void epi_channels(const EpiArgs &p, unsigned int i, unsigned int (&c)[4])
+{
+    if (PER4) {
         const unsigned int plane = magic_div(i, p.m_hw, p.s_hw);
-        const unsigned int c = plane - magic_div(plane, p.m_chan, p.s_chan) * p.channels;
-        const float v = __ldg(p.b + c);
-        return make_float4(v, v, v, v);
+        c[0] = c[1] = c[2] = c[3] = plane - magic_div(plane, p.m_chan, p.s_chan) * p.channels;
+        return;
     }
     const unsigned int e = 4u * i;
     const unsigned int plane = magic_div(e, p.m_hw, p.s_hw);
     unsigned int rem = e - plane * p.hw;
-    unsigned int c = plane - magic_div(plane, p.m_chan, p.s_chan) * p.channels;
-    float v[4];
+    unsigned int ch = plane - magic_div(plane, p.m_chan, p.s_chan) * p.channels;
 #pragma unroll
     for (int j = 0; j < 4; ++j) {
-        v[j] = __ldg(p.b + c);
+        c[j] = ch;
         if (++rem == p.hw) {
             rem = 0;
-            if (++c == p.channels) c = 0;
-        }
-    }
-    return make_float4(v[0], v[1], v[2], v[3]);
+            if (++ch == p.channels) ch = 0;
+        }
+    }
+}
+
+template <bool PER4>
+__device__ __forceinline__ float4 gather4(const float *v, const unsigned int (&c)[4])
+{
+    if (PER4) {
+        const float x = __ldg(v + c[0]);
+        return make_float4(x, x, x, x);
+    }
+    return make_float4(__ldg(v + c[0]), __ldg(v + c[1]), __ldg(v + c[2]), __ldg(v + c[3]));
+}
+
+template <int MODE>
+__device__ __forceinline__ float4 epi_load_a(const EpiArgs &p, unsigned int i)
+{
+    return MODE == EPI_BIAS4 || MODE == EPI_BIAS1 ? __ldcs(reinterpret_cast<const float4 *>(p.a) + i)
+                                                  : ld_stream_f4(reinterpret_cast<const float4 *>(p.a) + i);
+}
+
+template <int MODE>
+__device__ __forceinline__ float4 epi_load_b(const EpiArgs &p, unsigned int i)
+{
+    if (MODE == EPI_BIAS4 || MODE == EPI_BIAS1) {
+        unsigned int c[4];
+        epi_channels<MODE == EPI_BIAS4>(p, i, c);
+        return gather4<MODE == EPI_BIAS4>(p.b, c);
+    }
+    return ld_stream_f4(reinterpret_cast<const float4 *>(p.b) + i);
+}
+
+template <int MODE>
+__device__ __forceinline__ void epi_operand_bias(const EpiArgs &p, unsigned int i, float4 &a, float4 &b,
+                                                 unsigned int &ma, unsigned int &mb)
+{
+    if (MODE != EPI_ADD_BIAS4 && MODE != EPI_ADD_BIAS1) return;
+    unsigned int c[4];
+    epi_channels<MODE == EPI_ADD_BIAS4>(p, i, c);
+    if (p.bias_a) a = add4(a, gather4<MODE == EPI_ADD_BIAS4>(p.bias_a, c));
+    if (p.bias_b) b = add4(b, gather4<MODE == EPI_ADD_BIAS4>(p.bias_b, c));
+    ma = absmax4(ma, a);
+    mb = absmax4(mb, b);
 }
 
 __device__ __forceinline__ void epi_store(const EpiArgs &p, unsigned int i, const float4 &a, const float4 &b,
                                           unsigned int &m)
 {
-    const float4 o = make_float4(__fadd_rn(a.x, b.x), __fadd_rn(a.y, b.y), __fadd_rn(a.z, b.z), __fadd_rn(a.w, b.w));
-    __stcs(reinterpret_cast<float4 *>(p.out) + i, o);
+    const float4 o = add4(a, b);
+    if (p.out) __stcs(reinterpret_cast<float4 *>(p.out) + i, o);
     if (p.relu_out)
         reinterpret_cast<float4 *>(p.relu_out)[i] = make_float4(relu_aten(o.x), relu_aten(o.y), relu_aten(o.z),
                                                                 relu_aten(o.w));
-    m = max(max(m, max(absbits(o.x), absbits(o.y))), max(absbits(o.z), absbits(o.w)));
+    m = absmax4(m, o);
 }
 
 template <int MODE>
@@ -313,7 +355,7 @@
     const unsigned int nvec = (unsigned int)(p.n >> 2);
     const unsigned int stride = gridDim.x * kStatThreads;
     unsigned int i = blockIdx.x * kStatThreads + threadIdx.x;
-    unsigned int m = 0;
+    unsigned int m = 0, ma = 0, mb = 0;
     for (; i + (kEpiUnroll - 1) * stride < nvec; i += kEpiUnroll * stride) {
         float4 a[kEpiUnroll], b[kEpiUnroll];
 #pragma unroll
@@ -321,20 +363,137 @@
 #pragma unroll
         for (int u = 0; u < kEpiUnroll; ++u) b[u] = epi_load_b<MODE>(p, i + u * stride);
 #pragma unroll
-        for (int u = 0; u < kEpiUnroll; ++u) epi_store(p, i + u * stride, a[u], b[u], m);
-    }
-    for (; i < nvec; i += stride) epi_store(p, i, epi_load_a<MODE>(p, i), epi_load_b<MODE>(p, i), m);
+        for (int u = 0; u < kEpiUnroll; ++u) {
+            epi_operand_bias<MODE>(p, i + u * stride, a[u], b[u], ma, mb);
+            epi_store(p, i + u * stride, a[u], b[u], m);
+        }
+    }
+    for (; i < nvec; i += stride) {
+        float4 a = epi_load_a<MODE>(p, i), b = epi_load_b<MODE>(p, i);
+        epi_operand_bias<MODE>(p, i, a, b, ma, mb);
+        epi_store(p, i, a, b, m);
+    }
     const unsigned long long t = ((unsigned long long)nvec << 2) + blockIdx.x * kStatThreads + threadIdx.x;
     if (t < p.n) {
-        float b;
-        if (MODE == EPI_ADD) b = p.b[t];
-        else b = __ldg(p.b + (unsigned int)((t / (MODE == EPI_BIAS4 ? 4ull * p.hw : p.hw)) % p.channels));
-        const float o = __fadd_rn(p.a[t], b);
-        p.out[t] = o;
+        const bool per4 = MODE == EPI_BIAS4 || MODE == EPI_ADD_BIAS4;
+        const unsigned int c = (unsigned int)((t / (per4 ? 4ull * p.hw : p.hw)) % p.channels);
+        float a = p.a[t], b;
+        if (MODE == EPI_BIAS4 || MODE == EPI_BIAS1) {
+            b = __ldg(p.b + c);
+        } else {
+            b = p.b[t];
+            if (MODE != EPI_ADD) {
+                if (p.bias_a) a = __fadd_rn(a, __ldg(p.bias_a + c));
+                if (p.bias_b) b = __fadd_rn(b, __ldg(p.bias_b + c));
+                ma = max(ma, absbits(a));
+                mb = max(mb, absbits(b));
+            }
+        }
+        const float o = __fadd_rn(a, b);
+        if (p.out) p.out[t] = o;
         if (p.relu_out) p.relu_out[t] = relu_aten(o);
         m = max(m, absbits(o));
     }
     if (p.max_slot) block_max_publish(m, s_warp, p.max_slot);
+    if (MODE == EPI_ADD_BIAS4 || MODE == EPI_ADD_BIAS1) {
+        if (p.max_a) block_max_publish(ma, s_warp, p.max_a);
+        if (p.max_b) block_max_publish(mb, s_warp, p.max_b);
+    }
+}
+
+__global__ void __launch_bounds__(kStatThreads)
+stem_pool_kernel(const float *__restrict__ y0, const float *__restrict__ bias, float *__restrict__ out,
+                 unsigned int *max_slot, unsigned int planes, unsigned int channels, int H, int W, int P, int Q)
+{
+    __shared__ unsigned int s_warp[kStatThreads / 32];
+    const unsigned int PQ = (unsigned int)(P * Q);
+    const unsigned int total = planes * PQ;
+    unsigned int m = 0;
+    for (unsigned int o = blockIdx.x * kStatThreads + threadIdx.x; o < total; o += gridDim.x * kStatThreads) {
+        const unsigned int plane = o / PQ;
+        const int pq = (int)(o - plane * PQ);
+        const int p = pq / Q, q = pq - p * Q;
+        const float b = __ldg(bias + plane % channels);
+        const float *src = y0 + (size_t)plane * (size_t)(H * W);
+        const int h0 = max(2 * p - 1, 0), h1 = min(2 * p + 2, H);
+        const int w0 = max(2 * q - 1, 0), w1 = min(2 * q + 2, W);
+        float best = -INFINITY;
+        for (int h = h0; h < h1; ++h)
+            for (int w = w0; w < w1; ++w) {
+                const float v = __fadd_rn(__ldg(src + h * W + w), b);
+                m = max(m, absbits(v));
+                const float r = relu_aten(v);
+                if (r > best || isnan(r)) best = r;
+            }
+        out[o] = best;
+    }
+    if (max_slot) block_max_publish(m, s_warp, max_slot);
+}
+
+struct SegBias {
+    const float *bias[PQ_MAX_SEGMENTS];
+    unsigned int hwq[PQ_MAX_SEGMENTS], channels[PQ_MAX_SEGMENTS];
+    unsigned int m_hw[PQ_MAX_SEGMENTS], m_chan[PQ_MAX_SEGMENTS];
+    unsigned char s_hw[PQ_MAX_SEGMENTS], s_chan[PQ_MAX_SEGMENTS], per4[PQ_MAX_SEGMENTS];
+};
+
+struct BiasView {
+    const float *bias;
+    unsigned int hwq, channels, m_hw, m_chan, head;
+    int s_hw, s_chan;
+    bool per4;
+};
+
+__device__ __forceinline__ BiasView bias_view(const SegBias &t, int s, unsigned int head)
+{
+    BiasView b;
+    b.bias = t.bias[s];
+    b.hwq = t.hwq[s];
+    b.channels = t.channels[s];
+    b.m_hw = t.m_hw[s];
+    b.m_chan = t.m_chan[s];
+    b.s_hw = t.s_hw[s];
+    b.s_chan = t.s_chan[s];
+    b.per4 = t.per4[s] != 0;
+    b.head = head;
+    return b;
+}
+
+__device__ __forceinline__ float4 add_seg_bias(const BiasView &b, const float4 &v, unsigned int vec)
+{
+    if (b.per4) {
+        const unsigned int plane = magic_div(vec, b.m_hw, b.s_hw);
+        const float x = __ldg(b.bias + (plane - magic_div(plane, b.m_chan, b.s_chan) * b.channels));
+        return add4(v, make_float4(x, x, x, x));
+    }
+    const unsigned int e = b.head + 4u * vec;
+    const unsigned int plane = magic_div(e, b.m_hw, b.s_hw);
+    unsigned int rem = e - plane * b.hwq;
+    unsigned int c = plane - magic_div(plane, b.m_chan, b.s_chan) * b.channels;
+    float x[4];
+#pragma unroll
+    for (int j = 0; j < 4; ++j) {
+        x[j] = __ldg(b.bias + c);
+        if (++rem == b.hwq) {
+            rem = 0;
+            if (++c == b.channels) c = 0;
+        }
+    }
+    return add4(v, make_float4(x[0], x[1], x[2], x[3]));
+}
+
+__device__ __forceinline__ float seg_scalar(const BiasView &b, const float *p, unsigned long long e)
+{
+    const float v = p[e];
+    if (!b.bias) return v;
+    const unsigned long long hw = b.per4 ? 4ull * b.hwq : b.hwq;
+    return __fadd_rn(v, __ldg(b.bias + (unsigned int)((e / hw) % b.channels)));
+}
+
+__device__ __forceinline__ float4 seg_load(const BiasView &b, const float4 *body, unsigned int vec)
+{
+    const float4 v = ld_stream_f4(body + vec);
+    return b.bias ? add_seg_bias(b, v, vec) : v;
 }
 
 struct HistDiv {
@@ -426,12 +585,13 @@
 
 template <bool ZERO_AWARE>
 __device__ __forceinline__ void hist_redo_vecs(unsigned int redo, unsigned int *mine, unsigned int mine_addr,
-                                               const float4 *psrc, const HistDiv &h)
+                                               const float4 *body, unsigned int pvec, const BiasView &bv,
+                                               const HistDiv &h)
 {
     while (redo) {
         const int slot = __ffs(redo) - 1;
         redo &= redo - 1;
-        const float4 w = psrc[threadIdx.x + slot * kStatThreads];
+        const float4 w = seg_load(bv, body, pvec + threadIdx.x + slot * kStatThreads);
         hist_redo<ZERO_AWARE>(mine, mine_addr, w.x, h);
         hist_redo<ZERO_AWARE>(mine, mine_addr, w.y, h);
         hist_redo<ZERO_AWARE>(mine, mine_addr, w.z, h);
@@ -439,13 +599,14 @@
     }
 }
 
-__device__ __forceinline__ bool hist_flagged_has_zero(unsigned int redo, const float4 *psrc)
+__device__ __forceinline__ bool hist_flagged_has_zero(unsigned int redo, const float4 *body, unsigned int pvec,
+                                                     const BiasView &bv)
 {
     bool z = false;
     while (redo) {
         const int slot = __ffs(redo) - 1;
         redo &= redo - 1;
-        const float4 w = psrc[threadIdx.x + slot * kStatThreads];
+        const float4 w = seg_load(bv, body, pvec + threadIdx.x + slot * kStatThreads);
         z = z || w.x == 0.0f || w.y == 0.0f || w.z == 0.0f || w.w == 0.0f;
     }
     return z;
@@ -455,7 +616,8 @@
 
 template <int COPIES, int VPT = kVecPerThread>
 __global__ void __launch_bounds__(kStatThreads, VPT <= 4 ? 6 : 4)
-hist_multi_kernel(const __grid_constant__ SegTable tab, unsigned long long *__restrict__ hist)
+hist_multi_kernel(const __grid_constant__ SegTable tab, const __grid_constant__ SegBias sb,
+                  unsigned long long *__restrict__ hist)
 {
     extern __shared__ unsigned int s_raw[];
     const unsigned int raw_addr = (unsigned int)__cvta_generic_to_shared(s_raw);
@@ -476,6 +638,7 @@
     bool zero_aware = false;
     while (c < c_end) {
         const SegGeom g = seg_geom(tab, seg);
+        const BiasView bv = bias_view(sb, seg, g.head);
         const float interval = tab.param[seg];
         const HistDiv hd = make_hist_div(interval);
         const unsigned int seg_first = seg ? tab.chunk_end[seg - 1] : 0;
@@ -487,24 +650,29 @@
             if (left >= (unsigned long long)kChunkVecs) {
 #pragma unroll 1
                 for (int part = 0; part < kVecPerThread / VPT; ++part) {
+                    const unsigned int pvec = (unsigned int)v0 + part * VPT * kStatThreads;
                     const float4 *psrc = src + part * VPT * kStatThreads;
                     float4 v[VPT];
 #pragma unroll
                     for (int i = 0; i < VPT; ++i) v[i] = ld_stream_f4(psrc + threadIdx.x + i * kStatThreads);
+                    if (bv.bias) {
+#pragma unroll
+                        for (int i = 0; i < VPT; ++i) v[i] = add_seg_bias(bv, v[i], pvec + threadIdx.x + i * kStatThreads);
+                    }
                     if (zero_aware) {
                         const unsigned int redo = hist_add_vecs<true, VPT>(mine_addr, trash_addr, v, hd);
-                        hist_redo_vecs<true>(redo, mine, mine_addr, psrc, hd);
+                        hist_redo_vecs<true>(redo, mine, mine_addr, g.body, pvec, bv, hd);
                     } else {
                         const unsigned int redo = hist_add_vecs<false, VPT>(mine_addr, trash_addr, v, hd);
                         bool many_zeros = false;
-                        if (__popc(redo) >= 3) many_zeros = hist_flagged_has_zero(redo, psrc);
+                        if (__popc(redo) >= 3) many_zeros = hist_flagged_has_zero(redo, g.body, pvec, bv);
                         zero_aware = __any_sync(0xffffffffu, many_zeros);
-                        hist_redo_vecs<false>(redo, mine, mine_addr, psrc, hd);
+                        hist_redo_vecs<false>(redo, mine, mine_addr, g.body, pvec, bv, hd);
                     }
                 }
             } else {
                 for (unsigned int i = threadIdx.x; i < (unsigned int)left; i += kStatThreads) {
-                    const float4 v = ld_stream_f4(src + i);
+                    const float4 v = seg_load(bv, g.body, (unsigned int)v0 + i);
                     hist_add_exact(mine, v.x, interval);
                     hist_add_exact(mine, v.y, interval);
                     hist_add_exact(mine, v.z, interval);
@@ -512,8 +680,9 @@
                 }
             }
             if (c == seg_first) {
-                if (threadIdx.x < g.head) hist_add_exact(mine, g.p[threadIdx.x], interval);
-                if (threadIdx.x < g.tail) hist_add_exact(mine, g.p[g.n - g.tail + threadIdx.x], interval);
+                if (threadIdx.x < g.head) hist_add_exact(mine, seg_scalar(bv, g.p, threadIdx.x), interval);
+                if (threadIdx.x < g.tail)
+                    hist_add_exact(mine, seg_scalar(bv, g.p, g.n - g.tail + threadIdx.x), interval);
             }
         }
         __syncthreads();
@@ -542,7 +711,8 @@
 }
 
 __global__ void __launch_bounds__(kStatThreads)
-hist_generic_kernel(const __grid_constant__ SegTable tab, int nbins, unsigned long long *__restrict__ hist)
+hist_generic_kernel(const __grid_constant__ SegTable tab, const __grid_constant__ SegBias sb, int nbins,
+                    unsigned long long *__restrict__ hist)
 {
     extern __shared__ unsigned int s_bins[];
     const unsigned int per = (tab.total_chunks + gridDim.x - 1) / gridDim.x;
@@ -554,19 +724,19 @@
     int seg = seg_of_chunk(tab, c);
     while (c < c_end) {
         const SegGeom g = seg_geom(tab, seg);
+        const BiasView bv = bias_view(sb, seg, g.head);
         const float interval = tab.param[seg];
         const unsigned int seg_first = seg ? tab.chunk_end[seg - 1] : 0;
         const unsigned int seg_last = min(tab.chunk_end[seg], c_end);
         for (; c < seg_last; ++c) {
             const unsigned long long v0 = (unsigned long long)(c - seg_first) * kChunkVecs;
-            const float4 *src = g.body + v0;
             const unsigned long long left = g.nvec > v0 ? g.nvec - v0 : 0;
             const unsigned int nv = left >= (unsigned long long)kChunkVecs ? (unsigned int)kChunkVecs : (unsigned int)left;
             for (unsigned int i = threadIdx.x; i < nv; i += 4 * kStatThreads) {
                 float4 v[4];
 #pragma unroll
                 for (int j = 0; j < 4; ++j)
-                    if (i + j * kStatThreads < nv) v[j] = ld_stream_f4(src + i + j * kStatThreads);
+                    if (i + j * kStatThreads < nv) v[j] = seg_load(bv, g.body, (unsigned int)v0 + i + j * kStatThreads);
 #pragma unroll
                 for (int j = 0; j < 4; ++j)
                     if (i + j * kStatThreads < nv) {
@@ -577,8 +747,9 @@
                     }
             }
             if (c == seg_first) {
-                if (threadIdx.x < g.head) hist_add_exact_n(s_bins, g.p[threadIdx.x], interval, nbins);
-                if (threadIdx.x < g.tail) hist_add_exact_n(s_bins, g.p[g.n - g.tail + threadIdx.x], interval, nbins);
+                if (threadIdx.x < g.head) hist_add_exact_n(s_bins, seg_scalar(bv, g.p, threadIdx.x), interval, nbins);
+                if (threadIdx.x < g.tail)
+                    hist_add_exact_n(s_bins, seg_scalar(bv, g.p, g.n - g.tail + threadIdx.x), interval, nbins);
             }
         }
         __syncthreads();
```

Result: faster. 3852 (median of 6 runs) (+4.0%).
